# zju3dv/EnvGS

Measured on AMD Instinct MI355X. Metric: train iters/s (fwd+bwd of the render hot path + Adam step, one 800x800 view per GPU per iter) + render Mpix/s, higher is better.
Workload: dtype f32

## Files before the change

envgs_amd/_lib.py:

```python
import ctypes
import os

import torch

HERE = os.path.dirname(os.path.abspath(__file__))
LIB_PATH = os.path.join(HERE, "libenvgs_hip.so")
_lib = None

c_void_p, c_int, c_uint32, c_size_t = ctypes.c_void_p, ctypes.c_int, ctypes.c_uint32, ctypes.c_size_t


class RasterCfg(ctypes.Structure):
    _fields_ = [("P", ctypes.c_int32), ("sh_degree", ctypes.c_int32), ("sh_coeffs", ctypes.c_int32),
                ("channels", ctypes.c_int32), ("width", ctypes.c_int32), ("height", ctypes.c_int32),
                ("bg_len", ctypes.c_int32), ("debug", ctypes.c_int32), ("scale_modifier", ctypes.c_float),
                ("tanfovx", ctypes.c_float), ("tanfovy", ctypes.c_float), ("feature_f16", ctypes.c_int32)]


class AdamTensor(ctypes.Structure):
    _fields_ = [("param", ctypes.c_void_p), ("grad", ctypes.c_void_p), ("exp_avg", ctypes.c_void_p), ("exp_avg_sq", ctypes.c_void_p),
                ("numel", ctypes.c_int64), ("lr", ctypes.c_float), ("step", ctypes.c_float)]


class RowsTensor(ctypes.Structure):
    _fields_ = [("src", ctypes.c_void_p), ("dst", ctypes.c_void_p), ("row_bytes", ctypes.c_int64)]


class GrowTensor(ctypes.Structure):
    _fields_ = [("src", ctypes.c_void_p), ("dst", ctypes.c_void_p), ("row_bytes", ctypes.c_int64), ("kind", ctypes.c_int32), ("reserved0", ctypes.c_int32)]


class DensifyPlanArgs(ctypes.Structure):
    _fields_ = ([("P", ctypes.c_int64), ("N", ctypes.c_int32), ("flags", ctypes.c_uint32)]
                + [(n, ctypes.c_float) for n in ("grad_threshold", "size_limit", "split_screen_threshold", "min_opacity", "min_gradient", "r")]
                + [(n, ctypes.c_void_p) for n in ("ga", "dn", "mr", "wa", "scal", "opac", "cls", "scan", "counters", "temp")]
                + [("temp_bytes", ctypes.c_size_t)])


class DensifyRewriteArgs(ctypes.Structure):
    _fields_ = ([("P", ctypes.c_int64), ("out_rows", ctypes.c_int64), ("n_samples", ctypes.c_int64), ("N", ctypes.c_int32), ("count", ctypes.c_int32),
                 ("ratio_n", ctypes.c_double), ("r", ctypes.c_float), ("reserved0", ctypes.c_uint32)]
                + [(n, ctypes.c_void_p) for n in ("cls", "scan", "counters", "scal", "rotation", "samples")]
                + [("tensors", ctypes.POINTER(GrowTensor))])


class TraceLists(ctypes.Structure):
    _fields_ = [("hit_lists", ctypes.c_void_p), ("hit_cnt", ctypes.c_void_p), ("n_used", ctypes.c_void_p), ("cap", ctypes.c_int32),
                ("surf_acc", ctypes.c_void_p), ("surf_cnt", ctypes.c_void_p), ("surf_off", ctypes.c_void_p),
                ("scan_temp", ctypes.c_void_p), ("scan_temp_bytes", ctypes.c_size_t), ("ray_keys", ctypes.c_void_p),
                ("ray_order", ctypes.c_void_p), ("ray_sort_temp", ctypes.c_void_p), ("ray_sort_temp_bytes", ctypes.c_size_t),
                ("records", ctypes.c_void_p),
                ("num_records", ctypes.c_uint64), ("hit_state", ctypes.c_void_p), ("entries", ctypes.c_void_p), ("pairs", ctypes.c_void_p),
                ("n_entries", ctypes.c_void_p), ("compact_rows", ctypes.c_uint64), ("row_off", ctypes.c_void_p), ("batch_rows", ctypes.c_void_p),
                ("row_blk", ctypes.c_void_p), ("sh_perm", ctypes.c_void_p), ("state_planes", ctypes.c_int32),
                ("sparse_hits", ctypes.c_void_p), ("sparse_cap", ctypes.c_uint64),
                ("defer_reduce", ctypes.c_uint32), ("reserved0", ctypes.c_uint32), ("bwd_order", ctypes.c_void_p)]


class TraceCfg(ctypes.Structure):
    _fields_ = [("P", ctypes.c_int32), ("num_rays", ctypes.c_int32), ("sh_degree", ctypes.c_int32),
                ("sh_coeffs", ctypes.c_int32), ("max_trace_depth", ctypes.c_int32), ("start_from_first", ctypes.c_int32),
                ("has_others", ctypes.c_int32), ("bg_len", ctypes.c_int32), ("debug", ctypes.c_int32),
                ("ray_h", ctypes.c_int32), ("ray_w", ctypes.c_int32),
                ("scale_modifier", ctypes.c_float), ("specular_threshold", ctypes.c_float), ("feature_f16", ctypes.c_int32)]


class SupervisorArgs(ctypes.Structure):
    _fields_ = ([("N", ctypes.c_int64), ("P", ctypes.c_int64), ("flags", ctypes.c_uint32), ("reserved0", ctypes.c_uint32),
                 ("weight", ctypes.c_float * 5), ("reserved1", ctypes.c_float)]
                + [(n, ctypes.c_void_p) for n in ("norm_map", "surf_norm_map", "acc_map", "dpt_map", "dist_map", "env_opacity", "prior", "msk", "R", "near_far")]
                + [(n, ctypes.c_int64) for n in ("norm_map_row", "norm_map_ch", "surf_norm_map_row", "surf_norm_map_ch", "acc_map_row", "dpt_map_row",
                                                 "dist_map_row", "env_opacity_row", "prior_row", "prior_ch", "msk_row")]
                + [(n, ctypes.c_void_p) for n in ("g_norm_map", "g_surf_norm_map", "g_acc_map", "g_dist_map", "g_env_opacity", "partial")])


class SurfelInputsArgs(ctypes.Structure):
    _fields_ = ([(n, ctypes.c_int32) for n in ("P", "sh_degree", "sh_coeffs", "spec_channels")]
                + [(n, ctypes.c_void_p) for n in ("xyz", "features_dc", "features_rest", "scaling", "rotation", "opacity", "specular", "roughness", "campos",
                                                  "scales", "rotations", "opacities", "specular_act", "roughness_act", "shs", "colors", "others", "vertices",
                                                  "clamped",
                                                  "g_scales", "g_rotations", "g_opacities", "g_specular_act", "g_roughness_act", "g_shs", "g_colors", "g_others",
                                                  "d_xyz", "d_features_dc", "d_features_rest", "d_scaling", "d_rotation", "d_opacity", "d_specular", "d_roughness")])


class TsdfVolume(ctypes.Structure):
    _fields_ = ([(n, ctypes.c_int32) for n in ("nx", "ny", "nz")] + [(n, ctypes.c_float) for n in ("ox", "oy", "oz", "voxel")]
                + [(n, ctypes.c_void_p) for n in ("tsdf", "weight", "rgb")])


class TsdfView(ctypes.Structure):
    _fields_ = [("depth", ctypes.c_void_p), ("rgb", ctypes.c_void_p), ("H", ctypes.c_int32), ("W", ctypes.c_int32),
                ("fx", ctypes.c_float), ("fy", ctypes.c_float), ("cx", ctypes.c_float), ("cy", ctypes.c_float),
                ("R", ctypes.c_float * 9), ("T", ctypes.c_float * 3), ("depth_max", ctypes.c_float), ("trunc", ctypes.c_float)]


class TsdfViews(ctypes.Structure):
    _fields_ = [("count", ctypes.c_int32), ("reserved0", ctypes.c_int32), ("v", TsdfView * 8)]


_P = c_void_p
SYMBOLS = {
    "envgs_raster_scan_temp_bytes": (c_size_t, [ctypes.c_int32]),
    "envgs_raster_sort_temp_bytes": (c_size_t, [c_uint32, ctypes.c_int32, ctypes.c_int32]),
    "envgs_raster_project": (c_int, [ctypes.POINTER(RasterCfg)] + [_P] * 15 + [_P, c_size_t, ctypes.POINTER(c_uint32), _P]),
    "envgs_raster_bin_and_render": (c_int, [ctypes.POINTER(RasterCfg), c_uint32] + [_P] * 7 + [_P, c_size_t] + [_P] * 7 + [_P]),
    "envgs_raster_render_audit": (c_int, [ctypes.POINTER(RasterCfg)] + [_P] * 11 + [ctypes.c_int32, _P, _P]),
    "envgs_raster_backward": (c_int, [ctypes.POINTER(RasterCfg), c_uint32] + [_P] * 29 + [_P]),
    "envgs_bvh_temp_bytes": (c_size_t, [ctypes.c_int32]),
    "envgs_bvh_node_floats": (c_size_t, [ctypes.c_int32]),
    "envgs_bvh_build": (c_int, [ctypes.c_int32, _P, _P, _P, _P, c_size_t, ctypes.c_int32, _P]),
    "envgs_bvh_refit": (c_int, [ctypes.c_int32, _P, _P, _P, _P, _P, c_size_t, ctypes.c_int32, _P]),
    "envgs_bvh_quality": (c_int, [ctypes.c_int32, _P, _P, _P]),
    "envgs_trace_ray_sort_temp_bytes": (c_size_t, [ctypes.c_int32]),
    "envgs_trace_ray_order": (c_int, [ctypes.c_int32, _P, _P, _P, ctypes.c_int32, _P, _P, _P, c_size_t, _P]),
    "envgs_trace_forward": (c_int, [ctypes.POINTER(TraceCfg)] + [_P] * 22 + [ctypes.POINTER(TraceLists), _P]),
    "envgs_trace_backward": (c_int, [ctypes.POINTER(TraceCfg)] + [_P] * 35 + [ctypes.POINTER(TraceLists), _P]),
    "envgs_trace_backward_join": (c_int, [_P]),
    "envgs_sh_colors_forward": (c_int, [ctypes.c_int32] * 4 + [_P] * 7 + [_P]),
    "envgs_sh_colors_backward": (c_int, [ctypes.c_int32] * 4 + [_P] * 9 + [_P]),
    "envgs_surfel_quads": (c_int, [ctypes.c_int32] + [_P] * 5 + [_P]),
    "envgs_blend_forward": (c_int, [ctypes.c_int32] * 3 + [_P] * 3 + [_P]),
    "envgs_blend_backward": (c_int, [ctypes.c_int32] * 3 + [_P] * 5 + [_P]),
    "envgs_bounce_rays_forward": (c_int, [ctypes.c_int32] + [_P] * 8 + [_P]),
    "envgs_bounce_rays_backward": (c_int, [ctypes.c_int32] + [_P] * 13 + [_P]),
    "envgs_bounce_blend_forward": (c_int, [ctypes.c_int32] + [_P] * 5 + [_P]),
    "envgs_bounce_blend_backward": (c_int, [ctypes.c_int32] + [_P] * 8 + [_P]),
    "envgs_bounce_pack_mid": (c_int, [ctypes.c_int32, _P, ctypes.c_int32, ctypes.c_int32] + [_P] * 8 + [_P]),
    "envgs_reflect_forward": (c_int, [ctypes.c_int32, ctypes.c_int32, ctypes.c_float] + [_P] * 8 + [_P]),
    "envgs_reflect_backward": (c_int, [ctypes.c_int32, ctypes.c_int32, ctypes.c_float] + [_P] * 11 + [_P]),
    "envgs_select_acc": (c_int, [ctypes.c_int32, ctypes.c_int32, ctypes.c_float, _P, _P, _P]),
    "envgs_reflect_filtered_forward": (c_int, [ctypes.c_int32, ctypes.c_int32, ctypes.c_float, ctypes.c_int32] + [_P] * 10 + [_P]),
    "envgs_reflect_filtered_backward": (c_int, [ctypes.c_int32, ctypes.c_int32, ctypes.c_float, ctypes.c_int32] + [_P] * 13 + [_P]),
    "envgs_blend_filtered_forward": (c_int, [ctypes.c_int32] * 4 + [_P] * 6 + [_P]),
    "envgs_blend_filtered_backward": (c_int, [ctypes.c_int32] * 4 + [_P] * 7 + [_P]),
    "envgs_surface_normal_forward": (c_int, [ctypes.c_int32, ctypes.c_int32, ctypes.c_float, ctypes.c_float, ctypes.c_float] + [_P] * 4 + [_P]),
    "envgs_surface_normal_backward": (c_int, [ctypes.c_int32, ctypes.c_int32, ctypes.c_float, ctypes.c_float, ctypes.c_float] + [_P] * 5 + [_P]),
    "envgs_surfel_inputs_forward": (c_int, [ctypes.POINTER(SurfelInputsArgs), _P]),
    "envgs_surfel_inputs_backward": (c_int, [ctypes.POINTER(SurfelInputsArgs), _P]),
    "envgs_fused_adam": (c_int, [ctypes.c_int32, ctypes.POINTER(AdamTensor), ctypes.c_float, ctypes.c_float, ctypes.c_float, _P]),
    "envgs_compact_temp_bytes": (ctypes.c_size_t, [ctypes.c_int64]),
    "envgs_compact_scan": (c_int, [ctypes.c_int64, _P, _P, _P, _P, ctypes.c_size_t, _P]),
    "envgs_compact_gather": (c_int, [ctypes.c_int32, ctypes.POINTER(RowsTensor), ctypes.c_int64, _P, _P, _P]),
    "envgs_compact_gather_rows": (c_int, [ctypes.c_int32, ctypes.POINTER(RowsTensor), ctypes.c_int64, ctypes.c_int64, _P, _P, _P]),
    "envgs_knn3_mean_dist2": (c_int, [ctypes.c_int32, _P, _P, _P]),
    "envgs_densify_stats": (c_int, [ctypes.c_int64, ctypes.c_int32] + [_P] * 8 + [_P]),
    "envgs_densify_plan_temp_bytes": (ctypes.c_size_t, [ctypes.c_int64]),
    "envgs_densify_plan": (c_int, [ctypes.POINTER(DensifyPlanArgs), _P]),
    "envgs_densify_split_stds": (c_int, [ctypes.c_int64, ctypes.c_int32] + [_P] * 5 + [ctypes.c_int64, _P]),
    "envgs_densify_rewrite": (c_int, [ctypes.POINTER(DensifyRewriteArgs), _P]),
    "envgs_weight_select_temp_bytes": (ctypes.c_size_t, []),
    "envgs_weight_select": (c_int, [ctypes.c_int64, _P, _P, ctypes.c_int32, ctypes.c_int64, ctypes.c_int64, _P, _P, _P, ctypes.c_size_t, _P]),
    "envgs_visibility_mask_temp_bytes": (ctypes.c_size_t, [ctypes.c_int64]),
    "envgs_visibility_mask": (c_int, [ctypes.c_int64, _P, _P, ctypes.c_int64, _P, _P, _P, _P, ctypes.c_size_t, _P]),
    "envgs_oversize_plan": (c_int, [ctypes.c_int64, c_uint32, ctypes.c_float, ctypes.c_float] + [_P] * 8 + [_P]),
    "envgs_tsdf_integrate": (c_int, [ctypes.POINTER(TsdfVolume), ctypes.POINTER(TsdfViews), ctypes.c_float, _P]),
    "envgs_mesh_temp_bytes": (c_size_t, [ctypes.c_int32] * 3),
    "envgs_mesh_count": (c_int, [ctypes.POINTER(TsdfVolume), ctypes.c_float, ctypes.c_float, _P, c_size_t, _P, _P]),
    "envgs_mesh_extract": (c_int, [ctypes.POINTER(TsdfVolume), ctypes.c_float, _P, c_size_t, c_uint32, c_uint32, _P, _P, _P, _P]),
    "envgs_mesh_components_temp_bytes": (c_size_t, [c_uint32, c_uint32]),
    "envgs_mesh_components": (c_int, [c_uint32, c_uint32, _P, _P, c_size_t] + [_P] * 5 + [_P]),
    "envgs_mesh_select_temp_bytes": (c_size_t, [c_uint32, c_uint32]),
    "envgs_mesh_select_count": (c_int, [c_uint32, c_uint32, _P, _P, _P, c_size_t, _P, _P]),
    "envgs_mesh_select_emit": (c_int, [c_uint32, c_uint32] + [_P] * 4 + [_P, c_size_t, c_uint32, c_uint32] + [_P] * 4 + [_P]),
    "envgs_l1_ssim_partial_count": (ctypes.c_int64, [ctypes.c_int32, ctypes.c_int32, ctypes.c_int32]),
    "envgs_l1_ssim_forward": (c_int, [ctypes.c_int32, ctypes.c_int32, ctypes.c_int32, _P, _P, _P, _P, _P]),
    "envgs_l1_ssim_backward": (c_int, [ctypes.c_int32, ctypes.c_int32, ctypes.c_int32, _P, _P, _P, _P, ctypes.c_float, ctypes.c_float, _P, _P]),
    "envgs_depth_percentiles_temp_bytes": (c_size_t, []),
    "envgs_depth_percentiles": (c_int, [ctypes.c_int64, _P, ctypes.c_int64, _P, _P, c_size_t, _P]),
    "envgs_supervisor_partial_count": (ctypes.c_int64, [ctypes.c_int64, ctypes.c_int64]),
    "envgs_supervisor_forward": (c_int, [ctypes.POINTER(SupervisorArgs), _P]),
    "envgs_supervisor_finish": (c_int, [ctypes.POINTER(SupervisorArgs), _P, _P]),
    "envgs_supervisor_backward": (c_int, [ctypes.c_int64, _P, _P, _P, _P]),
    "envgs_debug_set": (None, [ctypes.c_int32, ctypes.c_int32]),
    "envgs_debug_get": (ctypes.c_int32, [ctypes.c_int32]),
    "envgs_prof_enable": (None, [c_int]),
    "envgs_prof_select": (None, [ctypes.c_uint64]),
    "envgs_prof_read": (c_int, [c_int, ctypes.POINTER(ctypes.c_double), ctypes.POINTER(c_int)]),
    "envgs_prof_kernel_name": (ctypes.c_char_p, [c_int]),
}


LIB_DIAG_PATH = os.path.join(HERE, "libenvgs_hip_diag.so")
_libs = {}
_selected = {"kind": "product"}


def _open(path):
    if not os.path.exists(path):
        raise RuntimeError(
            "envgs_amd: %s is missing. Build it with `python -m envgs_amd.build` (hipcc, gfx950). "
            "There is no CPU fallback for the render-and-trace path." % path)
    lib = ctypes.CDLL(path)
    for name, (res, args) in SYMBOLS.items():
        fn = getattr(lib, name)
        fn.restype = res
        fn.argtypes = args
    return lib


def load():
    global _lib
    kind = _selected["kind"]
    lib = _libs.get(kind)
    if lib is None:
        lib = _libs[kind] = _open(LIB_PATH if kind == "product" else LIB_DIAG_PATH)
    _lib = lib
    return lib


def select(kind):
    if kind not in ("product", "diag"):
        raise ValueError(kind)
    old = _selected["kind"]
    _selected["kind"] = kind
    load()
    return old


def ptr(t):
    return None if t is None else ctypes.c_void_p(t.data_ptr())


def check(rc, what):
    if rc != 0:
        raise RuntimeError("envgs_amd: %s failed with code %d (%s)" % (
            what, rc, {-1: "bad argument", -2: "temp buffer too small"}.get(rc, "hipError_t")))
```

envgs_amd/csrc/common.h:

```cpp
#pragma once
#include <hip/hip_runtime.h>
#include <hip/hip_fp16.h>
#include <stdint.h>

#include "../../include/envgs_raster.h"
#include "prof.h"

namespace envgs {

constexpr int TILE = ENVGS_TILE;
constexpr int GEOM = ENVGS_GEOM_STRIDE;
constexpr int GREC = ENVGS_GRAD_STRIDE;
constexpr float NEAR_N = 0.2f;
constexpr float FAR_N = 100.0f;
constexpr float FILTER_SIZE = 0.707106f;
constexpr float FILTER_INV_SQ = 2.0f;
constexpr float ALPHA_CAP = 0.99f;
constexpr float ALPHA_MIN = 1.0f / 255.0f;
constexpr float T_EPS = 0.0001f;

struct Feat {
    const void *p;
    bool h;
    __device__ __forceinline__ float operator[](size_t i) const {
        return h ? __half2float(reinterpret_cast<const __half *>(p)[i]) : reinterpret_cast<const float *>(p)[i];
    }
    __device__ __forceinline__ Feat at(size_t i) const { return Feat{reinterpret_cast<const char *>(p) + i * (h ? 2 : 4), h}; }
};

#define ENVGS_CHECK_LAUNCH(cfg, stream)                                             \
    do {                                                                            \
        hipError_t e__ = hipGetLastError();                                         \
        if (e__ != hipSuccess) return (int)e__;                                     \
        if ((cfg)->debug) {                                                         \
            e__ = hipStreamSynchronize((hipStream_t)(stream));                      \
            if (e__ != hipSuccess) return (int)e__;                                 \
        }                                                                           \
    } while (0)

template <int CTRL, int ROW_MASK = 0xf, int BANK_MASK = 0xf, bool BOUND = true>
__device__ __forceinline__ float dpp_mov(float v) {
    return __builtin_bit_cast(float, __builtin_amdgcn_update_dpp(0, __builtin_bit_cast(int, v), CTRL, ROW_MASK, BANK_MASK, BOUND));
}

__device__ __forceinline__ float wave_sum(float v) {
    v += dpp_mov<0xB1>(v);
    v += dpp_mov<0x4E>(v);
    v += dpp_mov<0x141>(v);
    v += dpp_mov<0x140>(v);
    v += dpp_mov<0x142, 0xa, 0xf, false>(v);
    v += dpp_mov<0x143, 0xc, 0xf, false>(v);
    return __builtin_bit_cast(float, __builtin_amdgcn_readlane(__builtin_bit_cast(int, v), 63));
}


typedef unsigned envgs_u2 __attribute__((ext_vector_type(2)));

__device__ __forceinline__ float wave_reduce64(const float (&g)[64], const int lane)
{
    float z[32];
#pragma unroll
    for (int i = 0; i < 32; i++) {
        const envgs_u2 r = __builtin_amdgcn_permlane32_swap(__float_as_uint(g[i]), __float_as_uint(g[i + 32]), false, false);
        z[i] = __uint_as_float(r.x) + __uint_as_float(r.y);
    }
    float w[16];
#pragma unroll
    for (int k = 0; k < 16; k++) {
        const envgs_u2 q = __builtin_amdgcn_permlane16_swap(__float_as_uint(z[k]), __float_as_uint(z[k + 16]), false, false);
        w[k] = __uint_as_float(q.x) + __uint_as_float(q.y);
    }
    const bool b3 = lane & 8, b2 = lane & 4, b1 = lane & 2, b0 = lane & 1;
    float a[8];
#pragma unroll
    for (int k = 0; k < 8; k++) a[k] = (b3 ? w[k + 8] : w[k]) + dpp_mov<0x140>(b3 ? w[k] : w[k + 8]);
    float b[4];
#pragma unroll
    for (int k = 0; k < 4; k++) b[k] = (b2 ? a[k + 4] : a[k]) + dpp_mov<0x141>(b2 ? a[k] : a[k + 4]);
    float c[2];
#pragma unroll
    for (int k = 0; k < 2; k++) c[k] = (b1 ? b[k + 2] : b[k]) + dpp_mov<0x1B>(b1 ? b[k] : b[k + 2]);
    return (b0 ? c[1] : c[0]) + dpp_mov<0xB1>(b0 ? c[0] : c[1]);
}

template <int CTRL, int ROW_MASK = 0xf>
__device__ __forceinline__ float dpp_fill(float v, float ident) {
    return __builtin_bit_cast(float, __builtin_amdgcn_update_dpp(__builtin_bit_cast(int, ident), __builtin_bit_cast(int, v), CTRL, ROW_MASK, 0xf, false));
}
__device__ __forceinline__ float wave_scan_add(float v) {
    v += dpp_fill<0x111>(v, 0.f); v += dpp_fill<0x112>(v, 0.f); v += dpp_fill<0x114>(v, 0.f); v += dpp_fill<0x118>(v, 0.f);
    v += dpp_fill<0x142, 0xa>(v, 0.f);
    v += dpp_fill<0x143, 0xc>(v, 0.f);
    return v;
}
__device__ __forceinline__ float wave_scan_mul(float v) {
    v *= dpp_fill<0x111>(v, 1.f); v *= dpp_fill<0x112>(v, 1.f); v *= dpp_fill<0x114>(v, 1.f); v *= dpp_fill<0x118>(v, 1.f);
    v *= dpp_fill<0x142, 0xa>(v, 1.f);
    v *= dpp_fill<0x143, 0xc>(v, 1.f);
    return v;
}
__device__ __forceinline__ float wave_bcast(float v, int l) { return __builtin_bit_cast(float, __builtin_amdgcn_readlane(__builtin_bit_cast(int, v), l)); }

template <int N4>
__device__ __forceinline__ float wave_transpose_reduce(const float (&g)[4 * N4], const int lane)
{
    float z[2 * N4];
#pragma unroll
    for (int i = 0; i < 2 * N4; i++) {
        const envgs_u2 r = __builtin_amdgcn_permlane32_swap(__float_as_uint(g[i]), __float_as_uint(g[i + 2 * N4]), false, false);
        z[i] = __uint_as_float(r.x) + __uint_as_float(r.y);
    }
    float w[N4];
#pragma unroll
    for (int k = 0; k < N4; k++) {
        const envgs_u2 q = __builtin_amdgcn_permlane16_swap(__float_as_uint(z[k]), __float_as_uint(z[k + N4]), false, false);
        float v = __uint_as_float(q.x) + __uint_as_float(q.y);
        v += dpp_mov<0x128>(v);
        v += dpp_mov<0x124>(v);
        v += dpp_mov<0x122>(v);
        v += dpp_mov<0x121>(v);
        w[k] = v;
    }
    float out = w[0];
#pragma unroll
    for (int k = 1; k < N4; k++) out = ((lane & 15) == k) ? w[k] : out;
    return out;
}

__device__ __forceinline__ int lane_id() { return __builtin_amdgcn_mbcnt_hi(~0u, __builtin_amdgcn_mbcnt_lo(~0u, 0u)); }

__device__ __forceinline__ void atomic_add_f32(float *p, float v) { unsafeAtomicAdd(p, v); }

int launch_project(const envgs_raster_cfg *cfg, const float *means3D, const float *scales, const float *rotations,
                   const float *opacities, const float *shs, const float *transmat_precomp, const float *viewmatrix,
                   const float *projmatrix, const float *campos, float *geom, float *rgb, uint8_t *clamped,
                   int32_t *radii, uint32_t *tiles_touched, hipStream_t stream);
int launch_scan(const uint32_t *in, uint32_t *out, int n, void *temp, size_t temp_bytes, hipStream_t stream);
size_t scan_temp_bytes(int n);
size_t sort_temp_bytes(uint32_t n, int width, int height);
int launch_bin(const envgs_raster_cfg *cfg, uint32_t N, const float *geom, const int32_t *radii, uint64_t *tile_pairs,
               uint64_t *keys_sorted, uint32_t *point_list, void *bin_temp, size_t bin_temp_bytes, uint32_t *ranges, hipStream_t stream);
size_t key_sort_temp_bytes(int n);
int launch_key_sort(int n, const uint64_t *keys_in, uint64_t *keys_out, int top_bit, void *temp, size_t temp_bytes, hipStream_t stream);
size_t ray_sort_temp_bytes(int R);
int launch_ray_sort(int R, const float *ray_o, const float *ray_d, const float4 *nodes, int P, uint64_t *pairs, uint32_t *order, void *temp,
                    size_t temp_bytes, hipStream_t stream);
int launch_render_fwd(const envgs_raster_cfg *cfg, const uint32_t *ranges, const uint32_t *point_list, const float *geom,
                      const float *colors, const float *bg, float *out_color, float *allmap, float *final_T,
                      int32_t *n_contrib, float *weight, hipStream_t stream, uint8_t *audit_contrib = nullptr, int audit_lmax = 0, int colors_f16 = 0,
                      uint8_t *contrib_mask = nullptr, const uint8_t *audit_skip = nullptr);
int launch_render_bwd(const envgs_raster_cfg *cfg, const uint32_t *ranges, const uint32_t *point_list, const float *geom,
                      const float *colors, const float *bg, const float *final_T, const int32_t *n_contrib,
                      const float *dL_dcolor, const float *dL_dallmap, float *grad_rec, hipStream_t stream, int colors_f16 = 0,
                      const uint8_t *contrib_mask = nullptr);
int launch_project_bwd(const envgs_raster_cfg *cfg, const float *geom, const float *means3D, const float *scales,
                       const float *rotations, const float *shs, const uint8_t *clamped, const float *transmat_precomp,
                       const int32_t *radii, const float *viewmatrix, const float *projmatrix, const float *campos,
                       const float *grad_rec, float *dmeans3D, float *dmeans2D, float *dscales, float *drots, float *dshs,
                       float *dcolors, float *dopacities, float *dtransmat_precomp, hipStream_t stream);

int launch_sh_record_bwd(int P, int D, const float *means3D, const float *shs, const float *campos, const uint8_t *clamped, const int32_t *radii,
                         const float *grad_rec, float *dmeans3D, float *dshs, hipStream_t stream);

__host__ __device__ inline int tile_bits(int width, int height) {
    int tiles = ((width + TILE - 1) / TILE) * ((height + TILE - 1) / TILE);
    int b = 0;
    while ((1 << b) < tiles) b++;
    return b < 1 ? 1 : b;
}

}
```

envgs_amd/csrc/raster_api.hip:

```cpp
#include "common.h"

using namespace envgs;

extern "C" {

size_t envgs_raster_scan_temp_bytes(int32_t P) { return scan_temp_bytes(P); }

size_t envgs_raster_sort_temp_bytes(uint32_t N, int32_t width, int32_t height)
{
    return sort_temp_bytes(N, width, height);
}

static int check_cfg(const envgs_raster_cfg *cfg)
{
    if (!cfg) return ENVGS_ERR_BAD_ARG;
    if (cfg->channels != 3 && cfg->channels != 5 && cfg->channels != 7) return ENVGS_ERR_BAD_ARG;
    if (cfg->sh_degree < 0 || cfg->sh_degree > 3) return ENVGS_ERR_BAD_ARG;
    if (cfg->width <= 0 || cfg->height <= 0 || cfg->P < 0) return ENVGS_ERR_BAD_ARG;
    return 0;
}

int envgs_raster_project(const envgs_raster_cfg *cfg, const float *means3D, const float *scales, const float *rotations,
                         const float *opacities, const float *shs, const float *transmat_precomp,
                         const float *viewmatrix, const float *projmatrix, const float *campos, float *geom, float *rgb,
                         uint8_t *clamped, int32_t *radii, uint32_t *tiles_touched, uint32_t *offsets, void *scan_temp,
                         size_t scan_temp_bytes_, uint32_t *num_rendered_host, void *stream_)
{
    int rc = check_cfg(cfg);
    if (rc) return rc;
    if (num_rendered_host) *num_rendered_host = 0;
    if (cfg->P == 0) return 0;
    if (!means3D || !opacities || !viewmatrix || !projmatrix || !geom || !radii || !tiles_touched || !offsets) return ENVGS_ERR_BAD_ARG;
    if (!transmat_precomp && (!scales || !rotations)) return ENVGS_ERR_BAD_ARG;
    if (shs && (cfg->channels != 3 || !rgb || !clamped || !campos || cfg->sh_coeffs < (cfg->sh_degree + 1) * (cfg->sh_degree + 1))) return ENVGS_ERR_BAD_ARG;
    hipStream_t stream = (hipStream_t)stream_;
    rc = launch_project(cfg, means3D, scales, rotations, opacities, shs, transmat_precomp, viewmatrix, projmatrix, campos,
                        geom, rgb, clamped, radii, tiles_touched, stream);
    if (rc) return rc;
    if (scan_temp_bytes_ < scan_temp_bytes(cfg->P)) return ENVGS_ERR_TEMP_TOO_SMALL;
    rc = launch_scan(tiles_touched, offsets, cfg->P, scan_temp, scan_temp_bytes_, stream);
    if (rc) return rc;
    if (!num_rendered_host) return 0;
    hipError_t e = hipMemcpyAsync(num_rendered_host, offsets + (cfg->P - 1), sizeof(uint32_t), hipMemcpyDeviceToHost, stream);
    if (e != hipSuccess) return (int)e;
    e = hipStreamSynchronize(stream);
    return (int)e;
}

int envgs_raster_bin_and_render(const envgs_raster_cfg *cfg, uint32_t N, const float *geom, const int32_t *radii,
                                const float *colors, const float *bg, uint64_t *tile_pairs, uint64_t *keys_sorted, uint32_t *point_list,
                                void *bin_temp, size_t bin_temp_bytes_, uint32_t *ranges, float *out_color, float *allmap,
                                float *final_T, int32_t *n_contrib, float *weight, uint8_t *contrib_mask, void *stream_)
{
    int rc = check_cfg(cfg);
    if (rc) return rc;
    if (!ranges || !out_color || !allmap || !final_T || !n_contrib || !bg) return ENVGS_ERR_BAD_ARG;
    if (cfg->P > 0 && (!geom || !radii || !colors || !weight)) return ENVGS_ERR_BAD_ARG;
    if (N > 0 && (!tile_pairs || !point_list || !bin_temp)) return ENVGS_ERR_BAD_ARG;
    hipStream_t stream = (hipStream_t)stream_;
    rc = launch_bin(cfg, N, geom, radii, tile_pairs, keys_sorted, point_list, bin_temp, bin_temp_bytes_, ranges, stream);
    if (rc) return rc;
    return launch_render_fwd(cfg, ranges, point_list, geom, colors, bg, out_color, allmap, final_T, n_contrib, weight, stream, nullptr, 0,
                             (cfg->feature_f16 && cfg->sh_coeffs == 0) ? 1 : 0, contrib_mask);
}

int envgs_raster_render_audit(const envgs_raster_cfg *cfg, const float *geom, const float *colors, const float *bg,
                              const uint32_t *point_list, const uint32_t *ranges, float *out_color, float *allmap, float *final_T,
                              int32_t *n_contrib, float *weight, uint8_t *contrib, int32_t lmax, const uint8_t *skip_px, void *stream_)
{
    int rc = check_cfg(cfg);
    if (rc) return rc;
    if (!ranges || !out_color || !allmap || !final_T || !n_contrib || !bg || !contrib || lmax <= 0) return ENVGS_ERR_BAD_ARG;
    if (cfg->P > 0 && (!geom || !colors || !weight || !point_list)) return ENVGS_ERR_BAD_ARG;
    hipStream_t stream = (hipStream_t)stream_;
    hipError_t e = hipMemsetAsync(contrib, 0, (size_t)cfg->width * cfg->height * (size_t)lmax, stream);
    if (e != hipSuccess) return (int)e;
    return launch_render_fwd(cfg, ranges, point_list, geom, colors, bg, out_color, allmap, final_T, n_contrib, weight, stream, contrib, lmax,
                             (cfg->feature_f16 && cfg->sh_coeffs == 0) ? 1 : 0, nullptr, skip_px);
}

int envgs_raster_backward(const envgs_raster_cfg *cfg, uint32_t N, const float *geom, const float *colors, const float *bg,
                          const uint32_t *point_list, const uint32_t *ranges, const float *final_T,
                          const int32_t *n_contrib, const uint8_t *contrib_mask, const float *dL_dcolor, const float *dL_dallmap, const float *means3D,
                          const float *scales, const float *rotations, const float *shs, const uint8_t *clamped,
                          const float *transmat_precomp, const int32_t *radii, const float *viewmatrix,
                          const float *projmatrix, const float *campos, float *grad_rec, float *dmeans3D, float *dmeans2D,
                          float *dscales, float *drots, float *dshs, float *dcolors, float *dopacities,
                          float *dtransmat_precomp, void *stream_)
{
    int rc = check_cfg(cfg);
    if (rc) return rc;
    if (cfg->P == 0) return 0;
    if (!geom || !colors || !bg || !ranges || !final_T || !n_contrib || !grad_rec || !radii ||
        !dmeans2D || !dopacities || !viewmatrix || !projmatrix)
        return ENVGS_ERR_BAD_ARG;
    if (N > 0 && !point_list) return ENVGS_ERR_BAD_ARG;
    if (shs ? (!dshs || !clamped || !campos || !means3D) : !dcolors) return ENVGS_ERR_BAD_ARG;
    if (transmat_precomp ? !dtransmat_precomp : (!scales || !rotations || !means3D || !dmeans3D || !dscales || !drots)) return ENVGS_ERR_BAD_ARG;
    hipStream_t stream = (hipStream_t)stream_;
    rc = launch_render_bwd(cfg, ranges, point_list, geom, colors, bg, final_T, n_contrib, dL_dcolor, dL_dallmap, grad_rec, stream,
                           (cfg->feature_f16 && !shs) ? 1 : 0, contrib_mask);
    if (rc) return rc;
    return launch_project_bwd(cfg, geom, means3D, scales, rotations, shs, clamped, transmat_precomp, radii, viewmatrix,
                              projmatrix, campos, grad_rec, dmeans3D, dmeans2D, dscales, drots, dshs, dcolors, dopacities,
                              dtransmat_precomp, stream);
}

}
```

envgs_amd/csrc/raster_bin.hip:

```cpp
#include "common.h"
#include "ray_key.h"
#include "tile_sort.h"

namespace envgs {

template <int CTRL, int ROW_MASK = 0xf>
__device__ __forceinline__ uint32_t dpp_fill_u32(uint32_t v) {
    return (uint32_t)__builtin_amdgcn_update_dpp(0, (int)v, CTRL, ROW_MASK, 0xf, false);
}
__device__ __forceinline__ uint32_t wave_scan_add_u32(uint32_t v) {
    v += dpp_fill_u32<0x111>(v); v += dpp_fill_u32<0x112>(v); v += dpp_fill_u32<0x114>(v); v += dpp_fill_u32<0x118>(v);
    v += dpp_fill_u32<0x142, 0xa>(v);
    v += dpp_fill_u32<0x143, 0xc>(v);
    return v;
}

template <int NW>
__device__ __forceinline__ uint32_t block_exclusive_u32(uint32_t v, uint32_t *s_w, uint32_t &total)
{
    const int lane = lane_id(), wave = threadIdx.x >> 6;
    const uint32_t inc = wave_scan_add_u32(v);
    if (lane == 63) s_w[wave] = inc;
    __syncthreads();
    uint32_t before = 0, all = 0;
#pragma unroll
    for (int k = 0; k < NW; k++) { const uint32_t t = s_w[k]; all += t; before += (k < wave) ? t : 0u; }
    total = all;
    __syncthreads();
    return before + inc - v;
}

constexpr int SCAN_ITEMS = 1024;

size_t scan_temp_bytes(int n) { return sizeof(uint32_t) * (size_t)(((n > 0 ? n : 1) + SCAN_ITEMS - 1) / SCAN_ITEMS) + 64; }

__global__ void __launch_bounds__(256)
scan_block_sums(const uint32_t *__restrict__ in, uint32_t *__restrict__ sums, int n)
{
    __shared__ uint32_t s_w[5];
    const int base = blockIdx.x * SCAN_ITEMS + threadIdx.x * 4;
    uint32_t s = 0;
#pragma unroll
    for (int k = 0; k < 4; k++) s += (base + k < n) ? in[base + k] : 0u;
    uint32_t total;
    (void)block_exclusive_u32<4>(s, s_w, total);
    if (threadIdx.x == 0) sums[blockIdx.x] = total;
}

__global__ void __launch_bounds__(256)
scan_apply(const uint32_t *in, uint32_t *out, const uint32_t *__restrict__ sums, int n)
{
    __shared__ uint32_t s_w[5];
    uint32_t pre = 0;
    for (int k = threadIdx.x; k < (int)blockIdx.x; k += 256) pre += sums[k];
    uint32_t before;
    (void)block_exclusive_u32<4>(pre, s_w, before);
    const int base = blockIdx.x * SCAN_ITEMS + threadIdx.x * 4;
    uint32_t a[4];
#pragma unroll
    for (int k = 0; k < 4; k++) a[k] = (base + k < n) ? in[base + k] : 0u;
    a[1] += a[0]; a[2] += a[1]; a[3] += a[2];
    uint32_t total;
    const uint32_t ex = block_exclusive_u32<4>(a[3], s_w, total) + before;
#pragma unroll
    for (int k = 0; k < 4; k++) if (base + k < n) out[base + k] = ex + a[k];
}

int launch_scan(const uint32_t *in, uint32_t *out, int n, void *temp, size_t temp_bytes, hipStream_t stream)
{
    if (n <= 0) return 0;
    if (temp_bytes < scan_temp_bytes(n)) return ENVGS_ERR_TEMP_TOO_SMALL;
    ProfScope prof_(K_SCAN, stream);
    const int nb = (n + SCAN_ITEMS - 1) / SCAN_ITEMS;
    hipLaunchKernelGGL(scan_block_sums, dim3(nb), dim3(256), 0, stream, in, (uint32_t *)temp, n);
    hipLaunchKernelGGL(scan_apply, dim3(nb), dim3(256), 0, stream, in, out, (const uint32_t *)temp, n);
    return (int)hipGetLastError();
}

constexpr int BIN_ROWS_MAX = 512;
constexpr int BIN_SLICE_MIN = 1024;
constexpr int BIN_BAND = 16384;
constexpr int BIG_RECT = 32;
constexpr int SORT_LONG_N = 16384;
constexpr int SORT_LONG_WGS = 256;

struct BinPlan { int rows, slice, ntiles; };
static BinPlan bin_plan(int P, int W, int H)
{
    BinPlan p;
    p.ntiles = ((W + TILE - 1) / TILE) * ((H + TILE - 1) / TILE);
    int rows = (P + BIN_SLICE_MIN - 1) / BIN_SLICE_MIN;
    rows = rows < 1 ? 1 : (rows > BIN_ROWS_MAX ? BIN_ROWS_MAX : rows);
    p.slice = (((P + rows - 1) / rows + 255) / 256) * 256;
    p.rows = p.slice > 0 ? (P + p.slice - 1) / p.slice : 1;
    if (p.rows < 1) p.rows = 1;
    return p;
}

size_t sort_temp_bytes(uint32_t, int width, int height)
{
    const size_t ntiles = (size_t)((width + TILE - 1) / TILE) * ((height + TILE - 1) / TILE);
    return sizeof(uint32_t) * ((size_t)BIN_ROWS_MAX * ntiles + 3 * ntiles + 1 + 4) + 256;
}

__device__ __forceinline__ bool tile_rect(int i, int W, int H, const float *__restrict__ geom, const int32_t *__restrict__ radii,
                                          int &x0, int &y0, int &x1, int &y1, uint32_t &dbits)
{
    const int rad = radii[i];
    if (rad <= 0) return false;
    const float cx = geom[(size_t)i * GEOM + 9], cy = geom[(size_t)i * GEOM + 10];
    dbits = __float_as_uint(geom[(size_t)i * GEOM + 15]);
    const float radius = (float)rad;
    const int gx = (W + TILE - 1) / TILE, gy = (H + TILE - 1) / TILE;
    x0 = (int)((cx - radius) / (float)TILE); x0 = x0 < 0 ? 0 : (x0 > gx ? gx : x0);
    y0 = (int)((cy - radius) / (float)TILE); y0 = y0 < 0 ? 0 : (y0 > gy ? gy : y0);
    x1 = (int)((cx + radius + (float)(TILE - 1)) / (float)TILE); x1 = x1 < 0 ? 0 : (x1 > gx ? gx : x1);
    y1 = (int)((cy + radius + (float)(TILE - 1)) / (float)TILE); y1 = y1 < 0 ? 0 : (y1 > gy ? gy : y1);
    return x1 > x0 && y1 > y0;
}

struct SurfelRect { int x0, y0, x1, y1; uint32_t dbits; bool vis; };
__device__ __forceinline__ SurfelRect load_rect(int i, int g1, int W, int H, const float *__restrict__ geom, const int32_t *__restrict__ radii)
{
    SurfelRect r;
    r.x0 = r.y0 = r.x1 = r.y1 = 0; r.dbits = 0;
    r.vis = i < g1 && tile_rect(i, W, H, geom, radii, r.x0, r.y0, r.x1, r.y1, r.dbits);
    return r;
}

template <bool SCATTER>
__global__ void __launch_bounds__(256)
bin_pass(int P, int W, int H, int slice, int ntiles, const float *__restrict__ geom, const int32_t *__restrict__ radii,
         uint32_t *hist, const uint32_t *__restrict__ tile_start, uint64_t *__restrict__ pairs, uint32_t cap)
{
    extern __shared__ uint32_t s_bin[];
    const int gx = (W + TILE - 1) / TILE;
    const int g0 = blockIdx.x * slice, g1 = min(P, g0 + slice);
    uint32_t *row = hist + (size_t)blockIdx.x * ntiles;
    const int lane = lane_id();
    for (int band0 = 0; band0 < ntiles; band0 += BIN_BAND) {
        const int bn = min(BIN_BAND, ntiles - band0);
        SurfelRect cur = load_rect(g0 + (int)threadIdx.x, g1, W, H, geom, radii);
        for (int t = threadIdx.x; t < bn; t += 256) s_bin[t] = SCATTER ? tile_start[band0 + t] + row[band0 + t] : 0u;
        __syncthreads();
        auto visit = [&](int t, uint64_t pair) {
            t -= band0;
            if ((unsigned)t >= (unsigned)bn) return;
            const uint32_t slot = atomicAdd(&s_bin[t], 1u);
            if (SCATTER && slot < cap) pairs[slot] = pair;
        };
        for (int ib = g0; ib < g1; ib += 256) {
            const int i = ib + (int)threadIdx.x;
            const SurfelRect c = cur;
            cur = load_rect(i + 256, g1, W, H, geom, radii);
            const int x0 = c.x0, y0 = c.y0, x1 = c.x1, y1 = c.y1;
            const uint32_t dbits = c.dbits;
            const bool vis = c.vis;
            const uint64_t pair = ((uint64_t)dbits << 32) | (uint32_t)i;
            const bool big = vis && (x1 - x0) * (y1 - y0) > BIG_RECT;
            if (vis && !big)
                for (int y = y0; y < y1; y++)
                    for (int x = x0; x < x1; x++) visit(y * gx + x, pair);
            uint64_t m = __builtin_amdgcn_ballot_w64(big);
            while (m) {
                const int l = __builtin_ctzll(m);
                m &= m - 1;
                const int bx0 = __builtin_amdgcn_readlane(x0, l), by0 = __builtin_amdgcn_readlane(y0, l);
                const int bw = __builtin_amdgcn_readlane(x1, l) - bx0, bh = __builtin_amdgcn_readlane(y1, l) - by0;
                const uint64_t bp = ((uint64_t)(uint32_t)__builtin_amdgcn_readlane((int)dbits, l) << 32) | (uint32_t)__builtin_amdgcn_readlane(i, l);
                for (int k = lane; k < bw * bh; k += 64) visit((by0 + k / bw) * gx + bx0 + k % bw, bp);
            }
        }
        __syncthreads();
        if (!SCATTER)
            for (int t = threadIdx.x; t < bn; t += 256) row[band0 + t] = s_bin[t];
        __syncthreads();
    }
}

constexpr int CS_SEG = 16, CS_ROWS = BIN_ROWS_MAX / CS_SEG;
__global__ void __launch_bounds__(256)
bin_column_scan(int rows, int ntiles, uint32_t *hist, uint32_t *__restrict__ tile_count)
{
    __shared__ uint32_t s_seg[CS_SEG][16];
    const int tl = threadIdx.x & 15, seg = threadIdx.x >> 4;
    const int t = blockIdx.x * 16 + tl;
    const int per = (rows + CS_SEG - 1) / CS_SEG, r0 = seg * per;
    uint32_t v[CS_ROWS];
    uint32_t s = 0;
#pragma unroll
    for (int k = 0; k < CS_ROWS; k++) {
        const int r = r0 + k;
        v[k] = (t < ntiles && k < per && r < rows) ? hist[(size_t)r * ntiles + t] : 0u;
        s += v[k];
    }
    s_seg[seg][tl] = s;
    __syncthreads();
    uint32_t acc = 0;
#pragma unroll
    for (int k = 0; k < CS_SEG; k++) acc += (k < seg) ? s_seg[k][tl] : 0u;
    if (t >= ntiles) return;
#pragma unroll
    for (int k = 0; k < CS_ROWS; k++) {
        const int r = r0 + k;
        if (k < per && r < rows) hist[(size_t)r * ntiles + t] = acc;
        acc += v[k];
    }
    if (seg == CS_SEG - 1) tile_count[t] = acc;
}

__global__ void __launch_bounds__(1024)
bin_tile_scan(int ntiles, const uint32_t *__restrict__ tile_count, uint32_t *__restrict__ tile_start, uint32_t *__restrict__ ranges,
              uint32_t cap, uint32_t *__restrict__ hdr)
{
    __shared__ uint32_t s_w[17];
    const int per = (ntiles + 1023) / 1024, b = min(ntiles, (int)threadIdx.x * per), e = min(ntiles, b + per);
    uint32_t s = 0;
    for (int k = b; k < e; k++) s += tile_count[k];
    uint32_t total;
    uint32_t run = block_exclusive_u32<16>(s, s_w, total);
    const bool ok = total <= cap;
    for (int k = b; k < e; k++) {
        const uint32_t c = tile_count[k];
        tile_start[k] = run;
        ranges[2 * k] = (c && ok) ? run : 0u;
        ranges[2 * k + 1] = (c && ok) ? run + c : 0u;
        run += c;
    }
    if (threadIdx.x == 0) { tile_start[ntiles] = total; hdr[0] = total; hdr[1] = 0u; hdr[2] = 0u; hdr[3] = 0u; }
}

template <int NT>
__device__ __forceinline__ void sort_padded_lds(uint64_t *s, int lp, int tid)
{
    const int npad = 1 << lp;
    for (int g = tid; g < (npad >> TS_S); g += NT) bitonic_first(s, g, lp);
    __syncthreads();
    for (int lk = TS_S + 1; lk <= lp; lk++)
        for (int a = lk - 1; a >= 0;) {
            const int S = ts_chunk(a);
            if (S == 4) { for (int g = tid; g < (npad >> 4); g += NT) bitonic_group<4>(s, g, lk, a, lp); }
            else if (S == 3) { for (int g = tid; g < (npad >> 3); g += NT) bitonic_group<3>(s, g, lk, a, lp); }
            else if (S == 2) { for (int g = tid; g < (npad >> 2); g += NT) bitonic_group<2>(s, g, lk, a, lp); }
            else { for (int g = tid; g < (npad >> 1); g += NT) bitonic_group<1>(s, g, lk, a, lp); }
            __syncthreads();
            a -= S;
        }
}

template <int NT>
__device__ __forceinline__ void merge_padded_lds(uint64_t *s, int lc, int tid)
{
    const int npad = 1 << lc;
    for (int a = lc - 1; a >= 0;) {
        const int S = ts_chunk(a);
        if (S == 4) { for (int g = tid; g < (npad >> 4); g += NT) bitonic_group<4>(s, g, lc, a, lc); }
        else if (S == 3) { for (int g = tid; g < (npad >> 3); g += NT) bitonic_group<3>(s, g, lc, a, lc); }
        else if (S == 2) { for (int g = tid; g < (npad >> 2); g += NT) bitonic_group<2>(s, g, lc, a, lc); }
        else { for (int g = tid; g < (npad >> 1); g += NT) bitonic_group<1>(s, g, lc, a, lc); }
        __syncthreads();
        a -= S;
    }
}

constexpr int lds_slots(int lp_cap) { return (1 << lp_cap) + (1 << (lp_cap - 5)); }

__device__ __forceinline__ void store_sorted(uint64_t v, uint32_t tile, size_t at, uint64_t *keys_sorted, uint32_t *point_list, int full64)
{
    if (full64) { keys_sorted[at] = v; return; }
    point_list[at] = (uint32_t)v;
    if (keys_sorted) keys_sorted[at] = ((uint64_t)tile << 32) | (v >> 32);
}

template <int NT>
__device__ __forceinline__ void load_sort_write(uint64_t *s, const uint64_t *pairs, int n, uint32_t tile, uint32_t b,
                                                uint64_t *keys_sorted, uint32_t *point_list, int tid, int full64)
{
    const int lp = ts_log2_padded(n);
    for (int i = tid; i < (1 << lp); i += NT) s[ts_slot(i)] = i < n ? pairs[b + i] : ~0ull;
    __syncthreads();
    sort_padded_lds<NT>(s, lp, tid);
    for (int i = tid; i < n; i += NT) store_sorted(s[ts_slot(i)], tile, (size_t)b + i, keys_sorted, point_list, full64);
}

template <int LP_CAP, int NT>
__global__ void __launch_bounds__(NT)
sort_tile_lists(const uint32_t *__restrict__ ranges, const uint64_t *pairs, uint64_t *keys_sorted, uint32_t *__restrict__ point_list,
                uint32_t *__restrict__ hdr, uint32_t *__restrict__ long_list, int full64)
{
    __shared__ uint64_t s_k[lds_slots(LP_CAP)];
    const uint32_t t = blockIdx.x, b = ranges[2 * t];
    const int n = (int)(ranges[2 * t + 1] - b);
    if (n == 0) return;
    if (n > (1 << LP_CAP)) {
        if (threadIdx.x == 0) long_list[atomicAdd(&hdr[1], 1u)] = t;
        return;
    }
    load_sort_write<NT>(s_k, pairs, n, t, b, keys_sorted, point_list, (int)threadIdx.x, full64);
}

constexpr int LONG_ITEM = 4096;
constexpr int LONG_BATCH = 256;

__device__ __forceinline__ uint32_t long_claim(uint32_t *hdr, uint32_t *s_item)
{
    __syncthreads();
    if (threadIdx.x == 0) *s_item = atomicAdd(&hdr[2], 1u);
    __syncthreads();
    return *s_item;
}
__device__ __forceinline__ void long_wait(uint32_t *hdr, const uint32_t base)
{
    if (threadIdx.x == 0)
        while (__hip_atomic_load(&hdr[3], __ATOMIC_ACQUIRE, __HIP_MEMORY_SCOPE_AGENT) < base) __builtin_amdgcn_s_sleep(4);
    __syncthreads();
    __threadfence();
}
__device__ __forceinline__ void long_done(uint32_t *hdr)
{
    __threadfence();
    __syncthreads();
    if (threadIdx.x == 0) __hip_atomic_fetch_add(&hdr[3], 1u, __ATOMIC_RELEASE, __HIP_MEMORY_SCOPE_AGENT);
}

__global__ void __launch_bounds__(1024)
sort_long_lists(const uint32_t *__restrict__ ranges, uint64_t *pairs, uint64_t *keys_sorted, uint32_t *__restrict__ point_list,
                uint32_t *hdr, const uint32_t *__restrict__ long_list, int full64)
{
    __shared__ uint64_t s_long[lds_slots(14)];
    __shared__ uint32_t s_item;
    __shared__ uint32_t s_bt[LONG_BATCH], s_bb[LONG_BATCH], s_bn[LONG_BATCH], s_pref[LONG_BATCH + 1];
    const uint32_t count = hdr[1];
    const int tid = (int)threadIdx.x, G = (int)gridDim.x;
    constexpr int LC = 14, C = 1 << LC;
    const bool copy_out = !(full64 && keys_sorted == pairs);
    uint32_t small_seen = 0u, big = 0u;
    for (uint32_t w = 0; w < count; w++) {
        const uint32_t t = long_list[w], b = ranges[2 * t];
        const int n = (int)(ranges[2 * t + 1] - b);
        if (n > SORT_LONG_N) { big++; continue; }
        if ((small_seen++ % (uint32_t)G) != blockIdx.x) continue;
        load_sort_write<1024>(s_long, pairs, n, t, b, keys_sorted, point_list, tid, full64);
        __syncthreads();
    }
    if (big == 0u) return;
    auto lp_of = [&](const int n) { int lp = LC; while ((1 << lp) < n) lp++; return lp; };
    auto items_of = [&](const int kind, const int lk, const int n) -> uint32_t {
        const int lp = lp_of(n);
        if (kind == 1) return lk <= lp ? (uint32_t)(((1ll << (lp - 1)) + LONG_ITEM - 1) / LONG_ITEM) : 0u;
        return (kind == 2 || lk <= lp) ? (uint32_t)((n + C - 1) / C) : 0u;
    };
    auto do_item = [&](const int kind, const int lk, const int q, const int l, const uint32_t it) {
        const uint32_t t = s_bt[l], b = s_bb[l];
        const int n = (int)s_bn[l];
        uint64_t *seg = pairs + b;
        if (kind == 0) {
            const int c = (int)it;
            for (int i = tid; i < C; i += 1024) s_long[ts_slot(i)] = ((long long)c * C + i) < n ? seg[(size_t)c * C + i] : ~0ull;
            __syncthreads();
            if (lk == LC) sort_padded_lds<1024>(s_long, LC, tid);
            else merge_padded_lds<1024>(s_long, LC, tid);
            for (int i = tid; i < C; i += 1024)
                if ((long long)c * C + i < n) seg[(size_t)c * C + i] = s_long[ts_slot(i)];
        } else if (kind == 1) {
            const int lp = lp_of(n);
            const long long i0 = (long long)it * LONG_ITEM, i1 = min(i0 + LONG_ITEM, 1ll << (lp - 1));
            for (long long idx = i0 + tid; idx < i1; idx += 1024) ascending_step(seg, n, lk, q, (int)idx);
        } else {
            const long long i0 = (long long)it * C, i1 = min(i0 + C, (long long)n);
            for (long long i = i0 + tid; i < i1; i += 1024) store_sorted(seg[i], t, (size_t)b + (size_t)i, keys_sorted, point_list, full64);
        }
    };
    uint32_t base = 0u, my = long_claim(hdr, &s_item);
    uint32_t w = 0;
    while (w < count) {
        __syncthreads();
        int nl = 0, lp_max = LC;
        for (; w < count && nl < LONG_BATCH; w++) {
            const uint32_t t = long_list[w], b = ranges[2 * t];
            const int n = (int)(ranges[2 * t + 1] - b);
            if (n <= SORT_LONG_N) continue;
            if (tid == 0) { s_bt[nl] = t; s_bb[nl] = b; s_bn[nl] = (uint32_t)n; }
            lp_max = max(lp_max, lp_of(n));
            nl++;
        }
        if (nl == 0) break;
        auto run_phase = [&](const int kind, const int lk, const int q) {
            __syncthreads();
            if (tid < nl) {
                uint32_t acc = 0u;
                for (int l = 0; l < tid; l++) acc += items_of(kind, lk, (int)s_bn[l]);
                s_pref[tid] = acc;
                if (tid == nl - 1) s_pref[nl] = acc + items_of(kind, lk, (int)s_bn[tid]);
            }
            __syncthreads();
            const uint32_t items = s_pref[nl];
            while (my - base < items) {
                const uint32_t j = my - base;
                int lo = 0, hi = nl - 1;
                while (lo < hi) { const int mid = (lo + hi + 1) >> 1; if (s_pref[mid] <= j) lo = mid; else hi = mid - 1; }
                long_wait(hdr, base);
                do_item(kind, lk, q, lo, j - s_pref[lo]);
                long_done(hdr);
                my = long_claim(hdr, &s_item);
            }
            base += items;
        };
        run_phase(0, LC, 0);
        for (int lk = LC + 1; lk <= lp_max; lk++) {
            for (int q = 0; q <= lk - LC - 1; q++) run_phase(1, lk, q);
            run_phase(0, lk, 0);
        }
        if (copy_out) run_phase(2, 0, 0);
    }
}

static int long_sort_grid()
{
    static int cached[16] = {};
    int dev = 0;
    if (hipGetDevice(&dev) != hipSuccess || dev < 0 || dev >= 16) return 64;
    if (cached[dev] == 0) {
        int cus = 0;
        if (hipDeviceGetAttribute(&cus, hipDeviceAttributeMultiprocessorCount, dev) != hipSuccess || cus <= 0) cus = 64;
        cached[dev] = cus < SORT_LONG_WGS ? cus : SORT_LONG_WGS;
    }
    return cached[dev];
}

int launch_bin(const envgs_raster_cfg *cfg, uint32_t N, const float *geom, const int32_t *radii, uint64_t *tile_pairs,
               uint64_t *keys_sorted, uint32_t *point_list, void *bin_temp, size_t bin_temp_bytes, uint32_t *ranges, hipStream_t stream)
{
    const BinPlan pl = bin_plan(cfg->P, cfg->width, cfg->height);
    if (N == 0 || cfg->P <= 0) return (int)hipMemsetAsync(ranges, 0, sizeof(uint32_t) * 2 * (size_t)pl.ntiles, stream);
    if (bin_temp_bytes < sort_temp_bytes(N, cfg->width, cfg->height)) return ENVGS_ERR_TEMP_TOO_SMALL;
    uint32_t *hist = (uint32_t *)bin_temp;
    uint32_t *tile_count = hist + (size_t)BIN_ROWS_MAX * pl.ntiles;
    uint32_t *tile_start = tile_count + pl.ntiles;
    uint32_t *long_list = tile_start + pl.ntiles + 1;
    uint32_t *hdr = long_list + pl.ntiles;
    const size_t lds = sizeof(uint32_t) * (size_t)(pl.ntiles < BIN_BAND ? pl.ntiles : BIN_BAND);
    prof_begin(K_EMIT_KEYS, stream);
    hipLaunchKernelGGL(bin_pass<false>, dim3(pl.rows), dim3(256), lds, stream, cfg->P, cfg->width, cfg->height, pl.slice, pl.ntiles,
                       geom, radii, hist, (const uint32_t *)nullptr, (uint64_t *)nullptr, 0u);
    ENVGS_CHECK_LAUNCH(cfg, stream);
    hipLaunchKernelGGL(bin_column_scan, dim3((pl.ntiles + 15) / 16), dim3(256), 0, stream, pl.rows, pl.ntiles, hist, tile_count);
    ENVGS_CHECK_LAUNCH(cfg, stream);
    hipLaunchKernelGGL(bin_tile_scan, dim3(1), dim3(1024), 0, stream, pl.ntiles, tile_count, tile_start, ranges, N, hdr);
    ENVGS_CHECK_LAUNCH(cfg, stream);
    hipLaunchKernelGGL(bin_pass<true>, dim3(pl.rows), dim3(256), lds, stream, cfg->P, cfg->width, cfg->height, pl.slice, pl.ntiles,
                       geom, radii, hist, tile_start, tile_pairs, N);
    ENVGS_CHECK_LAUNCH(cfg, stream);
    prof_end(K_EMIT_KEYS, stream);
    ProfScope prof_(K_SORT, stream);
    const uint64_t want = (uint64_t)N * 8 / ((uint64_t)pl.ntiles * 5);
    if (want <= 2048)
        hipLaunchKernelGGL((sort_tile_lists<11, 128>), dim3(pl.ntiles), dim3(128), 0, stream, ranges, tile_pairs, keys_sorted, point_list, hdr, long_list, 0);
    else if (want <= 4096)
        hipLaunchKernelGGL((sort_tile_lists<12, 256>), dim3(pl.ntiles), dim3(256), 0, stream, ranges, tile_pairs, keys_sorted, point_list, hdr, long_list, 0);
    else
        hipLaunchKernelGGL((sort_tile_lists<13, 512>), dim3(pl.ntiles), dim3(512), 0, stream, ranges, tile_pairs, keys_sorted, point_list, hdr, long_list, 0);
    ENVGS_CHECK_LAUNCH(cfg, stream);
    hipLaunchKernelGGL(sort_long_lists, dim3(long_sort_grid()), dim3(1024), 0, stream, ranges, tile_pairs,
                       keys_sorted, point_list, hdr, long_list, 0);
    ENVGS_CHECK_LAUNCH(cfg, stream);
    return 0;
}

static void launch_bucket_sorts(uint64_t n, int nb, const uint32_t *ranges, uint64_t *pairs, uint64_t *keys_sorted, uint32_t *point_list,
                                uint32_t *hdr, uint32_t *long_list, int full64, hipStream_t stream)
{
    const uint64_t want = n * 8 / ((uint64_t)nb * 5);
    if (want <= 2048)
        hipLaunchKernelGGL((sort_tile_lists<11, 128>), dim3(nb), dim3(128), 0, stream, ranges, pairs, keys_sorted, point_list, hdr, long_list, full64);
    else if (want <= 4096)
        hipLaunchKernelGGL((sort_tile_lists<12, 256>), dim3(nb), dim3(256), 0, stream, ranges, pairs, keys_sorted, point_list, hdr, long_list, full64);
    else
        hipLaunchKernelGGL((sort_tile_lists<13, 512>), dim3(nb), dim3(512), 0, stream, ranges, pairs, keys_sorted, point_list, hdr, long_list, full64);
    hipLaunchKernelGGL(sort_long_lists, dim3(long_sort_grid()), dim3(1024), 0, stream, ranges, pairs, keys_sorted, point_list, hdr, long_list, full64);
}

static int ray_bucket_bits(int R)
{
    int b = 4;
    while (b < 13 && ((long long)160 << b) < R) b++;
    return b;
}

size_t ray_sort_temp_bytes(int R)
{
    const size_t nb = (size_t)1 << ray_bucket_bits(R);
    return sizeof(uint32_t) * ((size_t)BIN_ROWS_MAX * nb + 5 * nb + 1 + 4 + (size_t)(R > 0 ? R : 1) + 6 * (size_t)BIN_ROWS_MAX) + 256;
}

__global__ void __launch_bounds__(256)
ray_origin_bounds(int R, int slice, const float *__restrict__ ray_o, float *__restrict__ partial)
{
    __shared__ float s_red[4][6];
    const int g0 = blockIdx.x * slice, g1 = min(R, g0 + slice);
    float lo[3] = {3.0e38f, 3.0e38f, 3.0e38f}, hi[3] = {-3.0e38f, -3.0e38f, -3.0e38f};
    for (int i = g0 + (int)threadIdx.x; i < g1; i += 256) {
#pragma unroll
        for (int c = 0; c < 3; c++) { const float x = ray_o[3 * i + c]; if (x == x && fabsf(x) < 1.0e30f) { lo[c] = fminf(lo[c], x); hi[c] = fmaxf(hi[c], x); } }
    }
#pragma unroll
    for (int c = 0; c < 3; c++)
        for (int o = 32; o > 0; o >>= 1) { lo[c] = fminf(lo[c], __shfl_xor(lo[c], o)); hi[c] = fmaxf(hi[c], __shfl_xor(hi[c], o)); }
    const int wave = threadIdx.x >> 6, lane = threadIdx.x & 63;
    if (lane == 0) { for (int c = 0; c < 3; c++) { s_red[wave][c] = lo[c]; s_red[wave][3 + c] = hi[c]; } }
    __syncthreads();
    if (threadIdx.x < 6) {
        const int c = threadIdx.x;
        float v = s_red[0][c];
        for (int w = 1; w < 4; w++) v = c < 3 ? fminf(v, s_red[w][c]) : fmaxf(v, s_red[w][c]);
        partial[blockIdx.x * 6 + c] = v;
    }
}

template <bool SCATTER>
__global__ void __launch_bounds__(256)
ray_bucket_pass(int R, int slice, int nb, int shift, const float *__restrict__ ray_o, const float *__restrict__ ray_d,
                const float *__restrict__ bounds_partial, int nrows, int lead, uint32_t *__restrict__ keys, uint32_t *hist, const uint32_t *__restrict__ bucket_start,
                uint64_t *__restrict__ pairs)
{
    extern __shared__ uint32_t s_bin[];
    __shared__ float s_box[6];
    const int g0 = blockIdx.x * slice, g1 = min(R, g0 + slice);
    uint32_t *row = hist + (size_t)blockIdx.x * nb;
    for (int t = threadIdx.x; t < nb; t += 256) s_bin[t] = SCATTER ? bucket_start[t] + row[t] : 0u;
    if (!SCATTER && threadIdx.x < 64) {
        const int c = threadIdx.x % 6, j0 = threadIdx.x / 6;
        float v = c < 3 ? 3.0e38f : -3.0e38f;
        if (j0 < 10)
            for (int j = j0; j < nrows; j += 10) { const float x = bounds_partial[j * 6 + c]; v = c < 3 ? fminf(v, x) : fmaxf(v, x); }
        float acc = v;
        for (int k = 1; k < 10; k++) { const float x = __shfl(v, (int)(threadIdx.x % 6) + 6 * k); if (threadIdx.x < 6) acc = c < 3 ? fminf(acc, x) : fmaxf(acc, x); }
        if (threadIdx.x < 6) s_box[c] = acc;
    }
    __syncthreads();
    float lo0 = 0.f, lo1 = 0.f, lo2 = 0.f, s0 = 0.f, s1 = 0.f, s2 = 0.f;
    if (!SCATTER) {
        lo0 = s_box[0]; lo1 = s_box[1]; lo2 = s_box[2];
        const float e0 = s_box[3] - lo0, e1 = s_box[4] - lo1, e2 = s_box[5] - lo2;
        s0 = e0 > 0.f ? 32.0f / e0 : 0.f; s1 = e1 > 0.f ? 32.0f / e1 : 0.f; s2 = e2 > 0.f ? 32.0f / e2 : 0.f;
    }
    for (int i = g0 + (int)threadIdx.x; i < g1; i += 256) {
        uint32_t key;
        if (SCATTER) key = keys[i];
        else keys[i] = key = ray_coherence_key(i, ray_o, ray_d, lo0, lo1, lo2, s0, s1, s2, lead);
        const uint32_t slot = atomicAdd(&s_bin[key >> shift], 1u);
        if (SCATTER) pairs[slot] = ((uint64_t)key << 32) | (uint32_t)i;
    }
    __syncthreads();
    if (!SCATTER)
        for (int t = threadIdx.x; t < nb; t += 256) row[t] = s_bin[t];
}

int launch_ray_sort(int R, const float *ray_o, const float *ray_d, const float4 *nodes, int P, uint64_t *pairs, uint32_t *order,
                    void *temp, size_t temp_bytes, hipStream_t stream)
{
    (void)nodes; (void)P;
    if (R <= 0) return 0;
    if (temp_bytes < ray_sort_temp_bytes(R)) return ENVGS_ERR_TEMP_TOO_SMALL;
    const int bits = ray_bucket_bits(R), nb = 1 << bits, shift = 31 - bits;
    int rows = (R + BIN_SLICE_MIN - 1) / BIN_SLICE_MIN;
    rows = rows < 1 ? 1 : (rows > BIN_ROWS_MAX ? BIN_ROWS_MAX : rows);
    const int slice = (((R + rows - 1) / rows + 255) / 256) * 256;
    rows = (R + slice - 1) / slice;
    uint32_t *hist = (uint32_t *)temp;
    uint32_t *count = hist + (size_t)BIN_ROWS_MAX * nb;
    uint32_t *start = count + nb;
    uint32_t *long_list = start + nb + 1;
    uint32_t *hdr = long_list + nb;
    uint32_t *ranges = hdr + 4;
    uint32_t *keys = ranges + 2 * (size_t)nb;
    float *partial = (float *)(keys + (size_t)R);
    const size_t lds = sizeof(uint32_t) * (size_t)nb;
    int lead = debug_switch(ENVGS_DBG_RAYKEY) > 0 ? debug_switch(ENVGS_DBG_RAYKEY) - 1 : RAY_KEY_LEAD;
    lead = lead > 8 ? 8 : lead;
    hipLaunchKernelGGL(ray_origin_bounds, dim3(rows), dim3(256), 0, stream, R, slice, ray_o, partial);
    hipLaunchKernelGGL(ray_bucket_pass<false>, dim3(rows), dim3(256), lds, stream, R, slice, nb, shift, ray_o, ray_d, (const float *)partial, rows, lead, keys, hist,
                       (const uint32_t *)nullptr, (uint64_t *)nullptr);
    hipLaunchKernelGGL(bin_column_scan, dim3((nb + 15) / 16), dim3(256), 0, stream, rows, nb, hist, count);
    hipLaunchKernelGGL(bin_tile_scan, dim3(1), dim3(1024), 0, stream, nb, count, start, ranges, (uint32_t)R, hdr);
    hipLaunchKernelGGL(ray_bucket_pass<true>, dim3(rows), dim3(256), lds, stream, R, slice, nb, shift, ray_o, ray_d, (const float *)partial, rows, lead, keys, hist, start, pairs);
    launch_bucket_sorts(R, nb, ranges, pairs, (uint64_t *)nullptr, order, hdr, long_list, 0, stream);
    return (int)hipGetLastError();
}

size_t key_sort_temp_bytes(int n)
{
    const size_t nb = (size_t)1 << ray_bucket_bits(n);
    return sizeof(uint32_t) * ((size_t)BIN_ROWS_MAX * nb + 5 * nb + 1 + 4) + 256;
}

template <bool SCATTER>
__global__ void __launch_bounds__(256)
key_bucket_pass(int n, int slice, int nb, int shift, const uint64_t *__restrict__ keys, uint32_t *hist, const uint32_t *__restrict__ bucket_start,
                uint64_t *__restrict__ out)
{
    extern __shared__ uint32_t s_bin[];
    const int g0 = blockIdx.x * slice, g1 = min(n, g0 + slice);
    uint32_t *row = hist + (size_t)blockIdx.x * nb;
    for (int t = threadIdx.x; t < nb; t += 256) s_bin[t] = SCATTER ? bucket_start[t] + row[t] : 0u;
    __syncthreads();
    for (int i = g0 + (int)threadIdx.x; i < g1; i += 256) {
        const uint64_t k = keys[i];
        const uint32_t slot = atomicAdd(&s_bin[(uint32_t)(k >> shift) & (uint32_t)(nb - 1)], 1u);
        if (SCATTER) out[slot] = k;
    }
    __syncthreads();
    if (!SCATTER)
        for (int t = threadIdx.x; t < nb; t += 256) row[t] = s_bin[t];
}

int launch_key_sort(int n, const uint64_t *keys_in, uint64_t *keys_out, int top_bit, void *temp, size_t temp_bytes, hipStream_t stream)
{
    if (n <= 0) return 0;
    if (temp_bytes < key_sort_temp_bytes(n)) return ENVGS_ERR_TEMP_TOO_SMALL;
    const int bits = ray_bucket_bits(n), nb = 1 << bits, shift = top_bit - bits;
    int rows = (n + BIN_SLICE_MIN - 1) / BIN_SLICE_MIN;
    rows = rows < 1 ? 1 : (rows > BIN_ROWS_MAX ? BIN_ROWS_MAX : rows);
    const int slice = (((n + rows - 1) / rows + 255) / 256) * 256;
    rows = (n + slice - 1) / slice;
    uint32_t *hist = (uint32_t *)temp;
    uint32_t *count = hist + (size_t)BIN_ROWS_MAX * nb;
    uint32_t *start = count + nb;
    uint32_t *long_list = start + nb + 1;
    uint32_t *hdr = long_list + nb;
    uint32_t *ranges = hdr + 4;
    const size_t lds = sizeof(uint32_t) * (size_t)nb;
    hipLaunchKernelGGL(key_bucket_pass<false>, dim3(rows), dim3(256), lds, stream, n, slice, nb, shift, keys_in, hist, (const uint32_t *)nullptr, (uint64_t *)nullptr);
    hipLaunchKernelGGL(bin_column_scan, dim3((nb + 15) / 16), dim3(256), 0, stream, rows, nb, hist, count);
    hipLaunchKernelGGL(bin_tile_scan, dim3(1), dim3(1024), 0, stream, nb, count, start, ranges, (uint32_t)n, hdr);
    hipLaunchKernelGGL(key_bucket_pass<true>, dim3(rows), dim3(256), lds, stream, n, slice, nb, shift, keys_in, hist, start, keys_out);
    launch_bucket_sorts((uint64_t)n, nb, ranges, keys_out, keys_out, (uint32_t *)nullptr, hdr, long_list, 1, stream);
    return (int)hipGetLastError();
}

}
```

envgs_amd/csrc/raster_render.hip:

```cpp
#include "common.h"

namespace envgs {

struct Hit {
    float sx, sy, inv, kx, ky, kz, lx, ly, lz, rho3d, rho2d, dx, dy, depth, G, alpha;
    bool ok;
};

template <bool EXACT>
__device__ __forceinline__ float recip(float x)
{
    if (EXACT) return 1.0f / x;
    const float r = __builtin_amdgcn_rcpf(x);
    return __builtin_fmaf(__builtin_fmaf(-x, r, 1.0f), r, r);
}
template <bool EXACT>
__device__ __forceinline__ float recip1(float x) { return EXACT ? 1.0f / x : __builtin_amdgcn_rcpf(x); }
template <bool EXACT>
__device__ __forceinline__ float expneg(float x) { return EXACT ? expf(x) : __expf(x); }

template <bool EXACT = false>
__device__ __forceinline__ Hit eval_splat(const float4 r0, const float4 r1, const float4 r2, const float4 r3, float px, float py)
{
    Hit h;
    const float Tux = r0.x, Tuy = r0.y, Tuz = r0.z, Tvx = r0.w, Tvy = r1.x, Tvz = r1.y, Twx = r1.z, Twy = r1.w, Twz = r2.x;
    const float cx = r2.y, cy = r2.z, opa = r3.z;
    h.kx = __builtin_fmaf(px, Twx, -Tux); h.ky = __builtin_fmaf(px, Twy, -Tuy); h.kz = __builtin_fmaf(px, Twz, -Tuz);
    h.lx = __builtin_fmaf(py, Twx, -Tvx); h.ly = __builtin_fmaf(py, Twy, -Tvy); h.lz = __builtin_fmaf(py, Twz, -Tvz);
    const float ppx = __builtin_fmaf(h.ky, h.lz, -(h.kz * h.ly));
    const float ppy = __builtin_fmaf(h.kz, h.lx, -(h.kx * h.lz));
    const float ppz = __builtin_fmaf(h.kx, h.ly, -(h.ky * h.lx));
    h.inv = recip<EXACT>(ppz);
    h.sx = ppx * h.inv; h.sy = ppy * h.inv;
    h.rho3d = __builtin_fmaf(h.sx, h.sx, h.sy * h.sy);
    h.dx = cx - px; h.dy = cy - py;
    h.rho2d = FILTER_INV_SQ * __builtin_fmaf(h.dx, h.dx, h.dy * h.dy);
    const bool use3d = h.rho3d <= h.rho2d;
    const float rho = use3d ? h.rho3d : h.rho2d;
    h.depth = use3d ? __builtin_fmaf(h.sx, Twx, __builtin_fmaf(h.sy, Twy, Twz)) : Twz;
    const float power = -0.5f * rho;
    h.G = expneg<EXACT>(power);
    const float a = opa * h.G;
    h.alpha = a < ALPHA_CAP ? a : ALPHA_CAP;
    h.ok = (ppz != 0.0f) && (h.depth >= NEAR_N) && (power <= 0.0f) && (h.alpha >= ALPHA_MIN);
    return h;
}

template <int C, int B = 256>
struct TileLds {
    float4 rec[4][B];
    float col[C][B];
    uint32_t id[B];
    unsigned long long qbits[4][(B + 63) / 64];
};

constexpr int BWD_BATCH = 192;

__device__ __forceinline__ int xcd_tile(int b, int ntiles)
{
    const int per = (ntiles + 7) >> 3;
    return (b & 7) * per + (b >> 3);
}

__device__ __forceinline__ uint32_t quadrant_mask(const float4 r0, const float4 r1, const float4 r2, const float4 r3, int tile_px, int tile_py)
{
    const float Tux = r0.x, Tuy = r0.y, Tuz = r0.z, Tvx = r0.w, Tvy = r1.x, Tvz = r1.y, Twx = r1.z, Twy = r1.w, Twz = r2.x;
    const float cx = r2.y, cy = r2.z, opa = r3.z;
    const float tau = 2.0f * __logf(255.0f * opa);
    if (!(tau >= 0.0f)) return 0u;
    const float r2d = sqrtf(0.5f * tau);
    float bx0 = cx - r2d, bx1 = cx + r2d, by0 = cy - r2d, by1 = cy + r2d;
    const float d = tau * (Twx * Twx + Twy * Twy) - Twz * Twz;
    if (!(d < 0.0f)) return 0xFu;
    const float id = 1.0f / d;
    const float f0 = tau * id, f2 = -id;
    const float pxc = f0 * (Tux * Twx + Tuy * Twy) + f2 * (Tuz * Twz);
    const float pyc = f0 * (Tvx * Twx + Tvy * Twy) + f2 * (Tvz * Twz);
    const float hx = pxc * pxc - (f0 * (Tux * Tux + Tuy * Tuy) + f2 * (Tuz * Tuz));
    const float hy = pyc * pyc - (f0 * (Tvx * Tvx + Tvy * Tvy) + f2 * (Tvz * Tvz));
    const float ex = sqrtf(fmaxf(hx, 0.0f)), ey = sqrtf(fmaxf(hy, 0.0f));
    bx0 = fminf(bx0, pxc - ex); bx1 = fmaxf(bx1, pxc + ex); by0 = fminf(by0, pyc - ey); by1 = fmaxf(by1, pyc + ey);
    const float mx = 0.05f + 1e-3f * (bx1 - bx0), my = 0.05f + 1e-3f * (by1 - by0);
    bx0 -= mx; bx1 += mx; by0 -= my; by1 += my;
    if (!(bx0 <= bx1 && by0 <= by1)) return 0xFu;
    const float ax = Tvy * Twz - Tvz * Twy, ay = Tvz * Twx - Tvx * Twz, az = Tvx * Twy - Tvy * Twx;
    const float bxx = Twy * Tuz - Twz * Tuy, bxy = Twz * Tux - Twx * Tuz, bxz = Twx * Tuy - Twy * Tux;
    const float A00 = ax * ax + ay * ay - tau * az * az, A11 = bxx * bxx + bxy * bxy - tau * bxz * bxz, A01 = ax * bxx + ay * bxy - tau * az * bxz;
    const float det = A00 * A11 - A01 * A01;
    const bool conic = A00 > 0.0f && A11 > 0.0f && det > 1e-6f * A00 * A11 && hx > 0.0f && hy > 0.0f &&
                       fabsf(hx * A00 - hy * A11) <= 0.02f * (hx * A00 + hy * A11);
    const float bound = conic ? 1.05f * hx * det / A11 : 0.0f;
    const float iA00 = conic ? 1.0f / A00 : 0.0f, iA11 = conic ? 1.0f / A11 : 0.0f;
    uint32_t m = 0;
#pragma unroll
    for (int q = 0; q < 4; q++) {
        const float qx = (float)(tile_px + (q & 1) * 8), qy = (float)(tile_py + (q >> 1) * 8);
        if (!(bx0 <= qx + 7.0f && bx1 >= qx && by0 <= qy + 7.0f && by1 >= qy)) continue;
        bool hit = true;
        if (conic) {
            const float ddx = fmaxf(fmaxf(qx - cx, cx - (qx + 7.0f)), 0.0f), ddy = fmaxf(fmaxf(qy - cy, cy - (qy + 7.0f)), 0.0f);
            const bool disc = ddx * ddx + ddy * ddy <= (r2d + 0.05f) * (r2d + 0.05f);
            const float x0 = qx - 0.05f - pxc, x1 = qx + 7.05f - pxc, y0 = qy - 0.05f - pyc, y1 = qy + 7.05f - pyc;
            bool ell = x0 <= 0.0f && x1 >= 0.0f && y0 <= 0.0f && y1 >= 0.0f;
            if (!ell) {
                float fmin = 3.0e38f;
#pragma unroll
                for (int e = 0; e < 2; e++) {
                    const float yy = e ? y1 : y0;
                    const float xs = fminf(fmaxf(-A01 * yy * iA00, x0), x1);
                    fmin = fminf(fmin, (A00 * xs + 2.0f * A01 * yy) * xs + A11 * yy * yy);
                    const float xx = e ? x1 : x0;
                    const float ys = fminf(fmaxf(-A01 * xx * iA11, y0), y1);
                    fmin = fminf(fmin, (A11 * ys + 2.0f * A01 * xx) * ys + A00 * xx * xx);
                }
                ell = fmin <= bound;
            }
            hit = disc || ell || !(bound == bound);
        }
        if (hit) m |= 1u << q;
    }
    return m;
}

template <int C, bool AUDIT, bool EXACT = false>
__global__ void __launch_bounds__(256, 5)
composite_fwd(int W, int H, int bg_len, const uint32_t *__restrict__ ranges, const uint32_t *__restrict__ point_list,
              const float *__restrict__ geom, const Feat colors, const float *__restrict__ bg,
              float *__restrict__ out_color, float *__restrict__ allmap, float *__restrict__ final_T,
              int32_t *__restrict__ n_contrib, float *__restrict__ weight, uint8_t *__restrict__ audit_contrib, int audit_lmax,
              uint8_t *__restrict__ contrib_mask, const uint8_t *__restrict__ audit_skip)
{
    __shared__ TileLds<C> lds;
    __shared__ float wacc[256];
    __shared__ unsigned char cmk[256][4];
    const int gx = (W + TILE - 1) / TILE, gy = (H + TILE - 1) / TILE;
    const int tile = xcd_tile(blockIdx.x, gx * gy);
    if (tile >= gx * gy) return;
    const int tx = tile % gx, ty = tile / gx;
    const int tid = threadIdx.x, wave = tid >> 6, lane = tid & 63;
    const int pxi = tx * TILE + (wave & 1) * 8 + (lane & 7);
    const int pyi = ty * TILE + (wave >> 1) * 8 + (lane >> 3);
    const bool inside = pxi < W && pyi < H;
    const float px = (float)pxi, py = (float)pyi;
    const uint32_t r0 = ranges[2 * tile], r1 = ranges[2 * tile + 1];

    const bool wskip = AUDIT && audit_skip && inside && audit_skip[(size_t)pyi * W + pxi] != 0;
    bool done = !inside;
    float T = 1.0f, Cacc[C], N0 = 0.f, N1 = 0.f, N2 = 0.f, D = 0.f, M1 = 0.f, M2 = 0.f, dist = 0.f, med = 0.f;
    int32_t last = 0, medc = -1;
#pragma unroll
    for (int c = 0; c < C; c++) Cacc[c] = 0.f;
    wacc[tid] = 0.f; reinterpret_cast<unsigned *>(&cmk[0][0])[tid] = 0u;

    for (uint32_t base = r0; base < r1; base += 256) {
        if (__syncthreads_and(done)) break;
        uint32_t qm = 0u;
        if (base + tid < r1) {
            const uint32_t g = point_list[base + tid];
            const float4 *gp = reinterpret_cast<const float4 *>(geom + (size_t)g * GEOM);
            const float4 a0 = gp[0], a1 = gp[1], a2 = gp[2], a3 = gp[3];
            lds.id[tid] = g;
            lds.rec[0][tid] = a0; lds.rec[1][tid] = a1; lds.rec[2][tid] = a2; lds.rec[3][tid] = a3;
            qm = quadrant_mask(a0, a1, a2, a3, tx * TILE, ty * TILE);
#pragma unroll
            for (int c = 0; c < C; c++) lds.col[c][tid] = colors[(size_t)g * C + c];
        }
#pragma unroll
        for (int q = 0; q < 4; q++) {
            const unsigned long long m = __builtin_amdgcn_ballot_w64((qm >> q) & 1u);
            if (lane == 0) lds.qbits[q][wave] = m;
        }
        __syncthreads();
        const int count = (int)min(256u, r1 - base);
        for (int ck = 0; ck * 64 < count && __builtin_amdgcn_ballot_w64(!done) != 0; ck++) {
          unsigned long long todo = lds.qbits[wave][ck];
          todo = ((unsigned long long)(unsigned)__builtin_amdgcn_readfirstlane((int)(todo >> 32)) << 32) | (unsigned)__builtin_amdgcn_readfirstlane((int)todo);
          while (todo != 0ull) {
            const int j = ck * 64 + (int)__builtin_ctzll(todo);
            todo &= todo - 1ull;
            if (__builtin_amdgcn_ballot_w64(!done) == 0) break;
            const Hit h = eval_splat<EXACT>(lds.rec[0][j], lds.rec[1][j], lds.rec[2][j], lds.rec[3][j], px, py);
            bool contrib = !done && h.ok;
            const float test_T = T * (1.0f - h.alpha);
            const bool stop = contrib && test_T < T_EPS;
            done = done || stop;
            contrib = contrib && !stop;
            float w = 0.f;
            if (contrib) {
                const float4 r2 = lds.rec[2][j], r3 = lds.rec[3][j];
                w = h.alpha * T;
                const float A = 1.0f - T;
                const float m = FAR_N / (FAR_N - NEAR_N) * (1.0f - NEAR_N / h.depth);
                dist += (m * m * A + M2 - 2.0f * m * M1) * w;
                D += h.depth * w;
                M1 += m * w;
                M2 += m * m * w;
                const int32_t contributor = (int32_t)(base - r0) + j + 1;
                if (AUDIT) { if (contributor <= audit_lmax) audit_contrib[((size_t)pyi * W + pxi) * (size_t)audit_lmax + (contributor - 1)] = 1; }
                if (T > 0.5f) { med = h.depth; medc = contributor; }
                N0 += r2.w * w; N1 += r3.x * w; N2 += r3.y * w;
#pragma unroll
                for (int c = 0; c < C; c++) Cacc[c] += lds.col[c][j] * w;
                T = test_T;
                last = contributor;
            }
            if (__builtin_amdgcn_ballot_w64(contrib) != 0) {
                const float ws = wave_sum((AUDIT && wskip) ? 0.f : w);
                if (lane == 0) { atomic_add_f32(&wacc[j], ws); cmk[j][wave] = 1; }
            }
          }
        }
        __syncthreads();
        if (tid < count) {
            const float ws = wacc[tid];
            if (ws != 0.0f) { atomic_add_f32(weight + lds.id[tid], ws); wacc[tid] = 0.f; }
            if (contrib_mask) {
                unsigned *cw = reinterpret_cast<unsigned *>(&cmk[0][0]) + tid;
                const unsigned v = *cw;
                contrib_mask[base + tid] = (uint8_t)((v & 1u) | ((v >> 7) & 2u) | ((v >> 14) & 4u) | ((v >> 21) & 8u));
                if (v) *cw = 0u;
            }
        }
    }

    if (inside) {
        const size_t HW = (size_t)H * W, pid = (size_t)pyi * W + pxi;
        final_T[pid] = T; final_T[HW + pid] = M1; final_T[2 * HW + pid] = M2;
        n_contrib[pid] = last; n_contrib[HW + pid] = medc;
#pragma unroll
        for (int c = 0; c < C; c++) out_color[c * HW + pid] = Cacc[c] + T * (c < bg_len ? bg[c] : 0.0f);
        allmap[0 * HW + pid] = D;
        allmap[1 * HW + pid] = 1.0f - T;
        allmap[2 * HW + pid] = N0; allmap[3 * HW + pid] = N1; allmap[4 * HW + pid] = N2;
        allmap[5 * HW + pid] = med;
        allmap[6 * HW + pid] = dist;
    }
}

template <int C, bool DIST, bool EXACT>
__device__ __forceinline__ void composite_bwd_tile(TileLds<C, BWD_BATCH> &lds, float (*gacc)[15 + C], const int W, const int H, const int bg_len,
                                                   const uint32_t *__restrict__ point_list, const float *__restrict__ geom,
                                                   const Feat colors, const float *__restrict__ bg,
                                                   const float *__restrict__ final_T, const int32_t *__restrict__ n_contrib,
                                                   const float *__restrict__ dL_dcolor, const float *__restrict__ dL_dallmap,
                                                   float *__restrict__ grad_rec, const uint32_t r0, const int tx, const int ty, const int max_last,
                                                   const uint8_t *__restrict__ contrib_mask)
{
    constexpr int V = 15 + C;
    constexpr int N4 = (V + 3) / 4;
    const int tid = threadIdx.x, wave = tid >> 6, lane = tid & 63;
    const int pxi = tx * TILE + (wave & 1) * 8 + (lane & 7);
    const int pyi = ty * TILE + (wave >> 1) * 8 + (lane >> 3);
    const bool inside = pxi < W && pyi < H;
    const float px = (float)pxi, py = (float)pyi;
    const size_t HW = (size_t)H * W, pid = (size_t)(inside ? pyi : 0) * W + (inside ? pxi : 0);

    const float T_final = inside ? final_T[pid] : 0.f;
    float T = T_final;
    const int32_t last = inside ? n_contrib[pid] : 0;
    const int32_t medc = inside ? n_contrib[HW + pid] : 0;
    float dpix[C];
    float bg_dot = 0.f;
#pragma unroll
    for (int c = 0; c < C; c++) {
        dpix[c] = (inside && dL_dcolor) ? dL_dcolor[c * HW + pid] : 0.f;
        bg_dot += (c < bg_len ? bg[c] : 0.0f) * dpix[c];
    }
    const float dL_ddepth = (inside && dL_dallmap) ? dL_dallmap[0 * HW + pid] : 0.f;
    const float dL_daccum = (inside && dL_dallmap) ? dL_dallmap[1 * HW + pid] : 0.f;
    const float dL_dn0 = (inside && dL_dallmap) ? dL_dallmap[2 * HW + pid] : 0.f;
    const float dL_dn1 = (inside && dL_dallmap) ? dL_dallmap[3 * HW + pid] : 0.f;
    const float dL_dn2 = (inside && dL_dallmap) ? dL_dallmap[4 * HW + pid] : 0.f;
    const float dL_dmed = (inside && dL_dallmap) ? dL_dallmap[5 * HW + pid] : 0.f;
    const float dL_dreg = (DIST && inside && dL_dallmap) ? dL_dallmap[6 * HW + pid] : 0.f;
    const float final_D = (DIST && inside) ? final_T[HW + pid] : 0.f;
    const float final_D2 = (DIST && inside) ? final_T[2 * HW + pid] : 0.f;
    const float final_A = 1.0f - T_final;
    const float bgT = -T_final * bg_dot;
    float last_alpha = 0.f, lastX = 0.f, accX = 0.f;
    int wmax_last = last;
    wmax_last = max(wmax_last, __shfl_xor(wmax_last, 1)); wmax_last = max(wmax_last, __shfl_xor(wmax_last, 2)); wmax_last = max(wmax_last, __shfl_xor(wmax_last, 4));
    wmax_last = max(wmax_last, __shfl_xor(wmax_last, 8)); wmax_last = max(wmax_last, __shfl_xor(wmax_last, 16)); wmax_last = max(wmax_last, __shfl_xor(wmax_last, 32));
    wmax_last = __builtin_amdgcn_readfirstlane(wmax_last);
    constexpr float MD_A = FAR_N / (FAR_N - NEAR_N), MD_B = (FAR_N * NEAR_N) / (FAR_N - NEAR_N);

    for (int top = max_last; top > 0; top -= BWD_BATCH) {
        __syncthreads();
        uint32_t qm = 0u;
        if (tid < BWD_BATCH && top - 1 - tid >= 0) {
            const uint32_t g = point_list[r0 + (uint32_t)(top - 1 - tid)];
            const float4 *gp = reinterpret_cast<const float4 *>(geom + (size_t)g * GEOM);
            const float4 a0 = gp[0], a1 = gp[1], a2 = gp[2], a3 = gp[3];
            lds.id[tid] = g;
            lds.rec[0][tid] = a0; lds.rec[1][tid] = a1; lds.rec[2][tid] = a2; lds.rec[3][tid] = a3;
            qm = contrib_mask ? (uint32_t)contrib_mask[r0 + (uint32_t)(top - 1 - tid)] : quadrant_mask(a0, a1, a2, a3, tx * TILE, ty * TILE);
#pragma unroll
            for (int c = 0; c < C; c++) lds.col[c][tid] = colors[(size_t)g * C + c];
        }
        if (wave * 64 < BWD_BATCH) {
#pragma unroll
            for (int q = 0; q < 4; q++) {
                const unsigned long long m = __builtin_amdgcn_ballot_w64((qm >> q) & 1u);
                if (lane == 0) lds.qbits[q][wave] = m;
            }
        }
        __syncthreads();
        const int count = min(BWD_BATCH, top);
        const int jmin = max(0, top - wmax_last);
        for (int ck = jmin >> 6; ck * 64 < count; ck++) {
          unsigned long long todo = lds.qbits[wave][ck];
          todo = ((unsigned long long)(unsigned)__builtin_amdgcn_readfirstlane((int)(todo >> 32)) << 32) | (unsigned)__builtin_amdgcn_readfirstlane((int)todo);
          if (ck == (jmin >> 6)) todo &= ~0ull << (jmin & 63);
          while (todo != 0ull) {
            const int j = ck * 64 + (int)__builtin_ctzll(todo);
            todo &= todo - 1ull;
            const int ci = top - 1 - j;
            const bool cand = ci < last;
            if (__builtin_amdgcn_ballot_w64(cand) == 0) continue;
            const float4 q0 = lds.rec[0][j], q1 = lds.rec[1][j], q2 = lds.rec[2][j], q3 = lds.rec[3][j];
            const Hit h = eval_splat<EXACT>(q0, q1, q2, q3, px, py);
            const bool act = cand && h.ok;
            if (__builtin_amdgcn_ballot_w64(act) == 0) continue;

            float gv[4 * N4];
#pragma unroll
            for (int v = 0; v < 4 * N4; v++) gv[v] = 0.f;
            if (act) {
                const float Twx = q1.z, Twy = q1.w, opa = q3.z;
                const float nrm0 = q2.w, nrm1 = q3.x, nrm2 = q3.y;
                const float alpha = h.alpha, G = h.G;
                const float r1 = recip1<EXACT>(1.0f - alpha);
                T = T * r1;
                const float w = alpha * T;
                float X = h.depth * dL_ddepth + dL_daccum;
                X += nrm0 * dL_dn0; X += nrm1 * dL_dn1; X += nrm2 * dL_dn2;
#pragma unroll
                for (int c = 0; c < C; c++) {
                    X += lds.col[c][j] * dpix[c];
                    gv[15 + c] = w * dpix[c];
                }
                float dL_dz = w * dL_ddepth;
                if (ci == medc - 1) dL_dz += dL_dmed;
                if (DIST) {
                    const float idep = recip1<EXACT>(h.depth);
                    const float m_d = MD_A * (1.0f - NEAR_N * idep);
                    X += (final_D2 + m_d * m_d * final_A - 2.0f * m_d * final_D) * dL_dreg;
                    dL_dz += 2.0f * w * (m_d * final_A - final_D) * dL_dreg * (MD_B * idep * idep);
                }
                accX = last_alpha * lastX + (1.f - last_alpha) * accX;
                lastX = X;
                last_alpha = alpha;
                const float dL_dalpha = (X - accX) * T + bgT * r1;
                gv[9] = w * dL_dn0; gv[10] = w * dL_dn1; gv[11] = w * dL_dn2;
                gv[12] = G * dL_dalpha;
                const float nGd = -(opa * dL_dalpha) * G;
                if (h.rho3d <= h.rho2d) {
                    const float dsx = __builtin_fmaf(nGd, h.sx, dL_dz * Twx);
                    const float dsy = __builtin_fmaf(nGd, h.sy, dL_dz * Twy);
                    const float dpx = dsx * h.inv, dpy = dsy * h.inv;
                    const float dpz = -__builtin_fmaf(dpx, h.sx, dpy * h.sy);
                    const float dkx = __builtin_fmaf(h.ly, dpz, -(h.lz * dpy)), dky = __builtin_fmaf(h.lz, dpx, -(h.lx * dpz)), dkz = __builtin_fmaf(h.lx, dpy, -(h.ly * dpx));
                    const float dlx = __builtin_fmaf(dpy, h.kz, -(dpz * h.ky)), dly = __builtin_fmaf(dpz, h.kx, -(dpx * h.kz)), dlz = __builtin_fmaf(dpx, h.ky, -(dpy * h.kx));
                    gv[0] = -dkx; gv[1] = -dky; gv[2] = -dkz;
                    gv[3] = -dlx; gv[4] = -dly; gv[5] = -dlz;
                    gv[6] = __builtin_fmaf(px, dkx, __builtin_fmaf(py, dlx, dL_dz * h.sx));
                    gv[7] = __builtin_fmaf(px, dky, __builtin_fmaf(py, dly, dL_dz * h.sy));
                    gv[8] = __builtin_fmaf(px, dkz, __builtin_fmaf(py, dlz, dL_dz));
                } else {
                    gv[13] = nGd * (FILTER_INV_SQ * h.dx);
                    gv[14] = nGd * (FILTER_INV_SQ * h.dy);
                    gv[8] = dL_dz;
                }
            }
            const float mine = wave_transpose_reduce<N4>(gv, lane);
            const int vi = (lane & 15) + (lane >> 4) * N4;
            if ((lane & 15) < N4 && vi < V) atomic_add_f32(&gacc[j][vi], mine);
          }
        }
        __syncthreads();
        for (int i = tid; i < count * V; i += 256) {
            const int j = i / V, v = i - j * V;
            const float val = gacc[j][v];
            if (val != 0.0f) { atomic_add_f32(grad_rec + (size_t)lds.id[j] * GREC + v, val); gacc[j][v] = 0.f; }
        }
    }
}

template <int C, bool EXACT = false>
__global__ void __launch_bounds__(256, 4)
composite_bwd(int W, int H, int bg_len, const uint32_t *__restrict__ ranges, const uint32_t *__restrict__ point_list,
              const float *__restrict__ geom, const Feat colors, const float *__restrict__ bg,
              const float *__restrict__ final_T, const int32_t *__restrict__ n_contrib,
              const float *__restrict__ dL_dcolor, const float *__restrict__ dL_dallmap, float *__restrict__ grad_rec,
              const uint8_t *__restrict__ contrib_mask)
{
    constexpr int V = 15 + C;
    __shared__ TileLds<C, BWD_BATCH> lds;
    __shared__ float gacc[BWD_BATCH][V];
    __shared__ int s_max_last, s_dist;
    const int gx = (W + TILE - 1) / TILE, gy = (H + TILE - 1) / TILE;
    const int tile = xcd_tile(blockIdx.x, gx * gy);
    if (tile >= gx * gy) return;
    const int tx = tile % gx, ty = tile / gx;
    const int tid = threadIdx.x, wave = tid >> 6, lane = tid & 63;
    const int pxi = tx * TILE + (wave & 1) * 8 + (lane & 7);
    const int pyi = ty * TILE + (wave >> 1) * 8 + (lane >> 3);
    const bool inside = pxi < W && pyi < H;
    const size_t HW = (size_t)H * W, pid = (size_t)(inside ? pyi : 0) * W + (inside ? pxi : 0);
    const int32_t last = inside ? n_contrib[pid] : 0;
    const bool reg = inside && dL_dallmap && dL_dallmap[6 * HW + pid] != 0.0f;

    if (tid == 0) { s_max_last = 0; s_dist = 0; }
    for (int i = tid; i < BWD_BATCH * V; i += 256) (&gacc[0][0])[i] = 0.f;
    __syncthreads();
    {
        int m = last;
        m = max(m, __shfl_xor(m, 1)); m = max(m, __shfl_xor(m, 2)); m = max(m, __shfl_xor(m, 4));
        m = max(m, __shfl_xor(m, 8)); m = max(m, __shfl_xor(m, 16)); m = max(m, __shfl_xor(m, 32));
        if (lane == 0) atomicMax(&s_max_last, m);
        const bool any_reg = __builtin_amdgcn_ballot_w64(reg) != 0;
        if (lane == 0 && any_reg) s_dist = 1;
    }
    __syncthreads();
    const int max_last = s_max_last;
    const uint32_t r0 = ranges[2 * tile];
    if (s_dist)
        composite_bwd_tile<C, true, EXACT>(lds, gacc, W, H, bg_len, point_list, geom, colors, bg, final_T, n_contrib, dL_dcolor, dL_dallmap, grad_rec, r0, tx, ty, max_last, contrib_mask);
    else
        composite_bwd_tile<C, false, EXACT>(lds, gacc, W, H, bg_len, point_list, geom, colors, bg, final_T, n_contrib, dL_dcolor, dL_dallmap, grad_rec, r0, tx, ty, max_last, contrib_mask);
}

template <int C>
static int run_fwd(const envgs_raster_cfg *cfg, const uint32_t *ranges, const uint32_t *point_list, const float *geom,
                   const float *colors, const float *bg, float *out_color, float *allmap, float *final_T,
                   int32_t *n_contrib, float *weight, uint8_t *audit_contrib, int audit_lmax, hipStream_t stream, int colors_f16, uint8_t *contrib_mask,
                   const uint8_t *audit_skip)
{
    const int gx = (cfg->width + TILE - 1) / TILE, gy = (cfg->height + TILE - 1) / TILE;
    ProfScope prof_(K_COMPOSITE_FWD, stream);
    const dim3 grid(8 * ((gx * gy + 7) / 8)), block(256);
    const Feat colors_{colors, colors_f16 != 0};
#ifdef ENVGS_DIAG
    if (debug_switch(ENVGS_DBG_RASTER_EXACT)) {
        if (audit_contrib)
            hipLaunchKernelGGL((composite_fwd<C, true, true>), grid, block, 0, stream, cfg->width, cfg->height, cfg->bg_len, ranges,
                               point_list, geom, colors_, bg, out_color, allmap, final_T, n_contrib, weight, audit_contrib, audit_lmax, contrib_mask, audit_skip);
        else
            hipLaunchKernelGGL((composite_fwd<C, false, true>), grid, block, 0, stream, cfg->width, cfg->height, cfg->bg_len, ranges,
                               point_list, geom, colors_, bg, out_color, allmap, final_T, n_contrib, weight, (uint8_t *)nullptr, 0, contrib_mask, (const uint8_t *)nullptr);
        ENVGS_CHECK_LAUNCH(cfg, stream);
        return 0;
    }
#endif
    if (audit_contrib)
        hipLaunchKernelGGL((composite_fwd<C, true>), grid, block, 0, stream, cfg->width, cfg->height, cfg->bg_len, ranges,
                           point_list, geom, colors_, bg, out_color, allmap, final_T, n_contrib, weight, audit_contrib, audit_lmax, contrib_mask, audit_skip);
    else
        hipLaunchKernelGGL((composite_fwd<C, false>), grid, block, 0, stream, cfg->width, cfg->height, cfg->bg_len, ranges,
                           point_list, geom, colors_, bg, out_color, allmap, final_T, n_contrib, weight, (uint8_t *)nullptr, 0, contrib_mask, (const uint8_t *)nullptr);
    ENVGS_CHECK_LAUNCH(cfg, stream);
    return 0;
}

int launch_render_fwd(const envgs_raster_cfg *cfg, const uint32_t *ranges, const uint32_t *point_list, const float *geom,
                      const float *colors, const float *bg, float *out_color, float *allmap, float *final_T,
                      int32_t *n_contrib, float *weight, hipStream_t stream, uint8_t *audit_contrib, int audit_lmax, int colors_f16, uint8_t *contrib_mask,
                      const uint8_t *audit_skip)
{
    if (cfg->P > 0) {
        hipError_t e = hipMemsetAsync(weight, 0, sizeof(float) * (size_t)cfg->P, stream);
        if (e != hipSuccess) return (int)e;
    }
    switch (cfg->channels) {
    case 3: return run_fwd<3>(cfg, ranges, point_list, geom, colors, bg, out_color, allmap, final_T, n_contrib, weight, audit_contrib, audit_lmax, stream, colors_f16, contrib_mask, audit_skip);
    case 5: return run_fwd<5>(cfg, ranges, point_list, geom, colors, bg, out_color, allmap, final_T, n_contrib, weight, audit_contrib, audit_lmax, stream, colors_f16, contrib_mask, audit_skip);
    case 7: return run_fwd<7>(cfg, ranges, point_list, geom, colors, bg, out_color, allmap, final_T, n_contrib, weight, audit_contrib, audit_lmax, stream, colors_f16, contrib_mask, audit_skip);
    default: return ENVGS_ERR_BAD_ARG;
    }
}

template <int C>
static int run_bwd(const envgs_raster_cfg *cfg, const uint32_t *ranges, const uint32_t *point_list, const float *geom,
                   const float *colors, const float *bg, const float *final_T, const int32_t *n_contrib,
                   const float *dL_dcolor, const float *dL_dallmap, float *grad_rec, hipStream_t stream, int colors_f16, const uint8_t *contrib_mask)
{
    const int gx = (cfg->width + TILE - 1) / TILE, gy = (cfg->height + TILE - 1) / TILE;
    ProfScope prof_(K_COMPOSITE_BWD, stream);
#ifdef ENVGS_DIAG
    if (debug_switch(ENVGS_DBG_RASTER_EXACT)) {
        hipLaunchKernelGGL((composite_bwd<C, true>), dim3(8 * ((gx * gy + 7) / 8)), dim3(256), 0, stream, cfg->width, cfg->height, cfg->bg_len, ranges,
                           point_list, geom, Feat{colors, colors_f16 != 0}, bg, final_T, n_contrib, dL_dcolor, dL_dallmap, grad_rec, contrib_mask);
        ENVGS_CHECK_LAUNCH(cfg, stream);
        return 0;
    }
#endif
    hipLaunchKernelGGL((composite_bwd<C, false>), dim3(8 * ((gx * gy + 7) / 8)), dim3(256), 0, stream, cfg->width, cfg->height, cfg->bg_len, ranges,
                       point_list, geom, Feat{colors, colors_f16 != 0}, bg, final_T, n_contrib, dL_dcolor, dL_dallmap, grad_rec, contrib_mask);
    ENVGS_CHECK_LAUNCH(cfg, stream);
    return 0;
}

int launch_render_bwd(const envgs_raster_cfg *cfg, const uint32_t *ranges, const uint32_t *point_list, const float *geom,
                      const float *colors, const float *bg, const float *final_T, const int32_t *n_contrib,
                      const float *dL_dcolor, const float *dL_dallmap, float *grad_rec, hipStream_t stream, int colors_f16, const uint8_t *contrib_mask)
{
    if (cfg->P <= 0) return 0;
    hipError_t e = hipMemsetAsync(grad_rec, 0, sizeof(float) * GREC * (size_t)cfg->P, stream);
    if (e != hipSuccess) return (int)e;
    switch (cfg->channels) {
    case 3: return run_bwd<3>(cfg, ranges, point_list, geom, colors, bg, final_T, n_contrib, dL_dcolor, dL_dallmap, grad_rec, stream, colors_f16, contrib_mask);
    case 5: return run_bwd<5>(cfg, ranges, point_list, geom, colors, bg, final_T, n_contrib, dL_dcolor, dL_dallmap, grad_rec, stream, colors_f16, contrib_mask);
    case 7: return run_bwd<7>(cfg, ranges, point_list, geom, colors, bg, final_T, n_contrib, dL_dcolor, dL_dallmap, grad_rec, stream, colors_f16, contrib_mask);
    default: return ENVGS_ERR_BAD_ARG;
    }
}

}
```

envgs_amd/raster.py:

```python
from typing import NamedTuple

import torch
from torch import nn

from . import _lib


LAST_STATS = {}


class GaussianRasterizationSettings(NamedTuple):
    image_height: int
    image_width: int
    tanfovx: float
    tanfovy: float
    bg: torch.Tensor
    scale_modifier: float
    viewmatrix: torch.Tensor
    projmatrix: torch.Tensor
    sh_degree: int
    campos: torch.Tensor
    prefiltered: bool
    debug: bool


def _f32c(t):
    if t is None:
        return None
    if t.dtype != torch.float32:
        t = t.float()
    return t.contiguous()


def _featc(t):
    if t is None:
        return None
    if t.dtype != torch.float16:
        return _f32c(t)
    return t.contiguous()


def _stream(dev):
    return _lib.c_void_p(torch.cuda.current_stream(dev).cuda_stream)


import weakref

_DEG_CACHE = {}


def sh_degree_of(deg):
    if not torch.is_tensor(deg):
        return int(deg)
    key = id(deg)
    hit = _DEG_CACHE.get(key)
    if hit is not None and hit[0]() is deg and hit[1] == deg._version:
        return hit[2]
    v = int(deg.reshape(-1)[0].item())
    if len(_DEG_CACHE) > 64:
        for k in [k for k, h in _DEG_CACHE.items() if h[0]() is None]:
            del _DEG_CACHE[k]
    _DEG_CACHE[key] = (weakref.ref(deg), deg._version, v)
    return v


SPECULATIVE_N = {"on": True}
_N_GUESS = {}
_N_MIRROR = {}


def _n_mirror(dev):
    m = _N_MIRROR.get(dev.index)
    if m is None:
        m = _N_MIRROR[dev.index] = dict(host=torch.empty(1, dtype=torch.int32).pin_memory(), event=torch.cuda.Event())
    return m


FEATURE_STORAGE = {"f16": False}


def _store(t):
    if t is not None and FEATURE_STORAGE["f16"] and t.dtype == torch.float32 and t.numel() > 0:
        return t.detach().half()
    return t


CONTRIB_MASK = {"on": True}


def _cfg(settings, P, C, sh_coeffs, bg_len, f16=False):
    deg = sh_degree_of(settings.sh_degree)
    return _lib.RasterCfg(P, deg, sh_coeffs, C, int(settings.image_width), int(settings.image_height), bg_len,
                          1 if settings.debug else 0, float(settings.scale_modifier), float(settings.tanfovx),
                          float(settings.tanfovy), 1 if f16 else 0)


def rasterize_forward(C, means3D, shs, colors_precomp, opacities, scales, rotations, cov3D_precomp, settings,
                      keep_binning=False):
    lib = _lib.load()
    dev = means3D.device
    if dev.type != "cuda":
        raise RuntimeError("envgs_amd rasterizer needs tensors on the GPU (got %s); there is no CPU path" % dev)
    P = means3D.shape[0]
    H, W = int(settings.image_height), int(settings.image_width)
    means3D = _f32c(means3D); opacities = _f32c(opacities)
    shs = _featc(shs); colors_precomp = _featc(colors_precomp)
    f16 = any(t is not None and t.dtype == torch.float16 for t in (shs, colors_precomp))
    scales = _f32c(scales); rotations = _f32c(rotations); cov3D_precomp = _f32c(cov3D_precomp)
    if shs is not None and C != 3:
        raise RuntimeError("in-kernel SH evaluation produces 3 channels; the %d-channel rasterizer needs colors_precomp" % C)
    if colors_precomp is not None and colors_precomp.shape[-1] != C:
        raise RuntimeError("colors_precomp has %d channels, this rasterizer composites %d" % (colors_precomp.shape[-1], C))
    bg = _f32c(settings.bg).reshape(-1).to(dev)
    view = _f32c(settings.viewmatrix).to(dev); proj = _f32c(settings.projmatrix).to(dev)
    campos = _f32c(settings.campos).reshape(-1).to(dev)
    sh_coeffs = 0 if shs is None else int(shs.shape[1])
    cfg = _cfg(settings, P, C, sh_coeffs, min(int(bg.numel()), C), f16)
    stream = _stream(dev)
    f32 = dict(dtype=torch.float32, device=dev)
    i32 = dict(dtype=torch.int32, device=dev)

    geom = torch.empty(P, 16, **f32)
    radii = torch.empty(P, **i32)
    tiles = torch.empty(P, **i32)
    offsets = torch.empty(P, **i32)
    rgb = torch.empty(P, 3, **f32) if shs is not None else None
    clamped = torch.empty(P, 3, dtype=torch.uint8, device=dev) if shs is not None else None
    scan_bytes = lib.envgs_raster_scan_temp_bytes(P)
    scan_temp = torch.empty(max(scan_bytes, 1), dtype=torch.uint8, device=dev)
    p = _lib.ptr
    tiles_n = ((W + 15) // 16) * ((H + 15) // 16)
    colors = rgb if shs is not None else colors_precomp
    out_color = torch.empty(C, H, W, **f32)
    allmap = torch.empty(7, H, W, **f32)
    final_T = torch.empty(3, H, W, **f32)
    n_contrib = torch.empty(2, H, W, **i32)
    weight = torch.empty(P, 1, **f32)
    ranges = torch.empty(tiles_n, 2, **i32)

    def bin_and_render(cap):
        pairs = torch.empty(max(cap, 1), dtype=torch.int64, device=dev)
        keys_s = torch.empty(max(cap, 1), dtype=torch.int64, device=dev) if keep_binning else None
        point_list = torch.empty(max(cap, 1), **i32)
        bin_bytes = lib.envgs_raster_sort_temp_bytes(max(cap, 1), W, H)
        bin_temp = torch.empty(max(bin_bytes, 1), dtype=torch.uint8, device=dev)
        cmask = torch.empty(max(cap, 1), dtype=torch.uint8, device=dev) if CONTRIB_MASK["on"] else None
        _lib.check(lib.envgs_raster_bin_and_render(cfg, cap, p(geom), p(radii), p(colors), p(bg), p(pairs), p(keys_s), p(point_list),
                                                   p(bin_temp), bin_bytes, p(ranges), p(out_color), p(allmap), p(final_T),
                                                   p(n_contrib), p(weight), p(cmask), stream),
                   "envgs_raster_bin_and_render")
        return pairs, keys_s, point_list, cmask

    key = (dev.index, P, H, W)
    guess = _N_GUESS.get(key) if SPECULATIVE_N["on"] else None
    mirror = _n_mirror(dev)
    if guess is None or P == 0:
        n_host = _lib.c_uint32(0)
        _lib.check(lib.envgs_raster_project(cfg, p(means3D), p(scales), p(rotations), p(opacities), p(shs), p(cov3D_precomp),
                                            p(view), p(proj), p(campos), p(geom), p(rgb), p(clamped), p(radii), p(tiles),
                                            p(offsets), p(scan_temp), scan_bytes, n_host, stream), "envgs_raster_project")
        N = int(n_host.value)
        bufs = bin_and_render(N)
    else:
        _lib.check(lib.envgs_raster_project(cfg, p(means3D), p(scales), p(rotations), p(opacities), p(shs), p(cov3D_precomp),
                                            p(view), p(proj), p(campos), p(geom), p(rgb), p(clamped), p(radii), p(tiles),
                                            p(offsets), p(scan_temp), scan_bytes, None, stream), "envgs_raster_project")
        mirror["host"].copy_(offsets[P - 1:P], non_blocking=True)
        mirror["event"].record(torch.cuda.current_stream(dev))
        cap = guess
        bufs = bin_and_render(cap)
        mirror["event"].synchronize()
        N = int(mirror["host"][0]) & 0xFFFFFFFF
        if N > cap:
            LAST_STATS["n_guess_misses"] = LAST_STATS.get("n_guess_misses", 0) + 1
            bufs = bin_and_render(N)
    pairs, keys_s, point_list, cmask = bufs
    _N_GUESS[key] = max(((max(int(N * 1.15), N + 4096) + 65535) // 65536) * 65536, int(0.97 * (guess or 0)))
    LAST_STATS.update(N=N, P=P, H=H, W=W, C=C)
    saved = dict(cfg=cfg, N=N, geom=geom, colors=colors, bg=bg, point_list=point_list, ranges=ranges, final_T=final_T,
                 n_contrib=n_contrib, contrib_mask=cmask, means3D=means3D, scales=scales, rotations=rotations, shs=shs, clamped=clamped,
                 cov3D_precomp=cov3D_precomp, radii=radii, view=view, proj=proj, campos=campos)
    if keep_binning:
        saved.update(tiles_touched=tiles, offsets=offsets, tile_pairs=pairs, keys_sorted=keys_s)
    return (out_color, radii, allmap, weight), saved


def render_audit(saved, lmax, skip_px=None, want_weight=False):
    lib = _lib.load()
    cfg = saved["cfg"]
    dev = saved["geom"].device
    H, W, C, P = cfg.height, cfg.width, cfg.channels, cfg.P
    f32 = dict(dtype=torch.float32, device=dev)
    out_color = torch.empty(C, H, W, **f32); allmap = torch.empty(7, H, W, **f32); final_T = torch.empty(3, H, W, **f32)
    n_contrib = torch.empty(2, H, W, dtype=torch.int32, device=dev); weight = torch.empty(max(P, 1), **f32)
    contrib = torch.empty(H * W, int(lmax), dtype=torch.uint8, device=dev)
    skip = None if skip_px is None else skip_px.to(device=dev, dtype=torch.uint8).reshape(-1).contiguous()
    if skip is not None and skip.numel() != H * W:
        raise RuntimeError("skip_px must have H*W elements")
    p = _lib.ptr
    _lib.check(lib.envgs_raster_render_audit(cfg, p(saved["geom"]), p(saved["colors"]), p(saved["bg"]), p(saved["point_list"]),
                                             p(saved["ranges"]), p(out_color), p(allmap), p(final_T), p(n_contrib), p(weight),
                                             p(contrib), int(lmax), p(skip), _stream(dev)), "envgs_raster_render_audit")
    if want_weight:
        return contrib, n_contrib, out_color, weight[:P]
    return contrib, n_contrib, out_color


def rasterize_backward(saved, dL_dcolor, dL_dallmap):
    lib = _lib.load()
    cfg = saved["cfg"]
    P, C = cfg.P, cfg.channels
    dev = saved["geom"].device
    f32 = dict(dtype=torch.float32, device=dev)
    dL_dcolor = _f32c(dL_dcolor); dL_dallmap = _f32c(dL_dallmap)
    shs, cov = saved["shs"], saved["cov3D_precomp"]
    grad_rec = torch.empty(P, 32, **f32)
    dmeans3D = torch.empty(P, 3, **f32)
    dmeans2D = torch.empty(P, 3, **f32)
    dopac = torch.empty(P, 1, **f32)
    dscales = torch.empty(P, 2, **f32) if cov is None else None
    drots = torch.empty(P, 4, **f32) if cov is None else None
    dcov = torch.empty(P, 9, **f32) if cov is not None else None
    dshs = torch.empty(shs.shape, **f32) if shs is not None else None
    dcolors = torch.empty(P, C, **f32) if shs is None else None
    p = _lib.ptr
    _lib.check(lib.envgs_raster_backward(cfg, saved["N"], p(saved["geom"]), p(saved["colors"]), p(saved["bg"]),
                                         p(saved["point_list"]), p(saved["ranges"]), p(saved["final_T"]), p(saved["n_contrib"]),
                                         p(saved.get("contrib_mask")), p(dL_dcolor), p(dL_dallmap), p(saved["means3D"]), p(saved["scales"]), p(saved["rotations"]),
                                         p(shs), p(saved["clamped"]), p(cov), p(saved["radii"]), p(saved["view"]), p(saved["proj"]),
                                         p(saved["campos"]), p(grad_rec), p(dmeans3D), p(dmeans2D), p(dscales), p(drots), p(dshs),
                                         p(dcolors), p(dopac), p(dcov), _stream(dev)), "envgs_raster_backward")
    return dict(means3D=dmeans3D, means2D=dmeans2D, shs=dshs, colors_precomp=dcolors, opacities=dopac, scales=dscales,
                rotations=drots, cov3D_precomp=dcov, grad_rec=grad_rec)


def make_package(C):

    class _RasterizeGaussians(torch.autograd.Function):
        @staticmethod
        def forward(ctx, means3D, means2D, sh, colors_precomp, opacities, scales, rotations, cov3Ds_precomp, raster_settings):
            ctx.set_materialize_grads(False)
            none = lambda t: None if (t is None or t.numel() == 0) else t
            outs, saved = rasterize_forward(C, means3D, _store(none(sh)), _store(none(colors_precomp)), opacities, none(scales),
                                            none(rotations), none(cov3Ds_precomp), raster_settings)
            ctx.saved = saved
            ctx.in_dtypes = tuple(None if t is None else t.dtype for t in (means3D, means2D, sh, colors_precomp, opacities, scales, rotations, cov3Ds_precomp))
            color, radii, allmap, weight = outs
            ctx.mark_non_differentiable(radii, weight)
            return color, radii, allmap, weight

        @staticmethod
        def backward(ctx, grad_color, grad_radii, grad_allmap, grad_weight):
            saved = ctx.saved
            cfg = saved["cfg"]
            dev = saved["geom"].device
            g = rasterize_backward(saved, grad_color, grad_allmap)
            outs = (g["means3D"] if saved["cov3D_precomp"] is None or saved["shs"] is not None else None, g["means2D"],
                    g["shs"], g["colors_precomp"], g["opacities"], g["scales"], g["rotations"], g["cov3D_precomp"])
            outs = tuple(None if (o is None or dt is None) else o.to(dt) for o, dt in zip(outs, ctx.in_dtypes))
            return outs + (None,)

    class GaussianRasterizer(nn.Module):
        def __init__(self, raster_settings):
            super().__init__()
            self.raster_settings = raster_settings

        def markVisible(self, positions):
            with torch.no_grad():
                V = self.raster_settings.viewmatrix.to(positions.device).float()
                z = positions.float() @ V[:3, 2] + V[3, 2]
                return z > 0.2

        def forward(self, means3D, means2D, opacities, shs=None, colors_precomp=None, scales=None, rotations=None,
                    cov3D_precomp=None):
            rs = self.raster_settings
            if (shs is None and colors_precomp is None) or (shs is not None and colors_precomp is not None):
                raise Exception('Please provide excatly one of either SHs or precomputed colors!')
            if ((scales is None or rotations is None) and cov3D_precomp is None) or \
               ((scales is not None or rotations is not None) and cov3D_precomp is not None):
                raise Exception('Please provide exactly one of either scale/rotation pair or precomputed 3D covariance!')
            e = torch.Tensor([])
            return _RasterizeGaussians.apply(means3D, means2D, e if shs is None else shs,
                                             e if colors_precomp is None else colors_precomp, opacities,
                                             e if scales is None else scales, e if rotations is None else rotations,
                                             e if cov3D_precomp is None else cov3D_precomp, rs)

    GaussianRasterizer.channels = C
    GaussianRasterizer._function = _RasterizeGaussians
    return GaussianRasterizationSettings, GaussianRasterizer
```

include/envgs_raster.h:

```cpp
#ifndef ENVGS_RASTER_H
#define ENVGS_RASTER_H

#include <stddef.h>
#include <stdint.h>

#ifdef __cplusplus
extern "C" {
#endif

#if defined(__GNUC__)
#define ENVGS_API __attribute__((visibility("default")))
#else
#define ENVGS_API
#endif

#define ENVGS_TILE 16
#define ENVGS_GEOM_STRIDE 16
#define ENVGS_GRAD_STRIDE 32

typedef enum envgs_status {
    ENVGS_OK = 0,
    ENVGS_ERR_BAD_ARG = -1,
    ENVGS_ERR_TEMP_TOO_SMALL = -2
} envgs_status;

typedef struct envgs_raster_cfg {
    int32_t P;
    int32_t sh_degree;
    int32_t sh_coeffs;
    int32_t channels;
    int32_t width, height;
    int32_t bg_len;
    int32_t debug;
    float scale_modifier;
    float tanfovx, tanfovy;
    int32_t feature_f16;
} envgs_raster_cfg;

ENVGS_API size_t envgs_raster_scan_temp_bytes(int32_t P);
ENVGS_API size_t envgs_raster_sort_temp_bytes(uint32_t N, int32_t width, int32_t height);

ENVGS_API int envgs_raster_project(const envgs_raster_cfg *cfg,
                         const float *means3D, const float *scales, const float *rotations,
                         const float *opacities, const float *shs, const float *transmat_precomp,
                         const float *viewmatrix, const float *projmatrix, const float *campos,
                         float *geom, float *rgb, uint8_t *clamped, int32_t *radii,
                         uint32_t *tiles_touched, uint32_t *offsets,
                         void *scan_temp, size_t scan_temp_bytes,
                         uint32_t *num_rendered_host, void *stream);

ENVGS_API int envgs_raster_bin_and_render(const envgs_raster_cfg *cfg, uint32_t N,
                                const float *geom, const int32_t *radii,
                                const float *colors, const float *bg,
                                uint64_t *tile_pairs, uint64_t *keys_sorted , uint32_t *point_list,
                                void *bin_temp, size_t bin_temp_bytes, uint32_t *ranges,
                                float *out_color, float *allmap, float *final_T, int32_t *n_contrib,
                                float *weight, uint8_t *contrib_mask, void *stream);

ENVGS_API int envgs_raster_render_audit(const envgs_raster_cfg *cfg, const float *geom, const float *colors, const float *bg,
                              const uint32_t *point_list, const uint32_t *ranges,
                              float *out_color, float *allmap, float *final_T, int32_t *n_contrib, float *weight,
                              uint8_t *contrib, int32_t lmax, const uint8_t *skip_px, void *stream);

ENVGS_API int envgs_raster_backward(const envgs_raster_cfg *cfg, uint32_t N,
                          const float *geom, const float *colors, const float *bg,
                          const uint32_t *point_list, const uint32_t *ranges,
                          const float *final_T, const int32_t *n_contrib, const uint8_t *contrib_mask ,
                          const float *dL_dcolor, const float *dL_dallmap,
                          const float *means3D, const float *scales, const float *rotations,
                          const float *shs, const uint8_t *clamped, const float *transmat_precomp,
                          const int32_t *radii,
                          const float *viewmatrix, const float *projmatrix, const float *campos,
                          float *grad_rec,
                          float *dmeans3D, float *dmeans2D, float *dscales, float *drots,
                          float *dshs, float *dcolors, float *dopacities, float *dtransmat_precomp,
                          void *stream);

ENVGS_API void envgs_prof_enable(int on);
ENVGS_API void envgs_prof_select(uint64_t kernel_mask);
ENVGS_API int envgs_prof_read(int kernel_id, double *total_ms, int *launches);
ENVGS_API const char *envgs_prof_kernel_name(int kernel_id);

#define ENVGS_DBG_TRACE 0
#define ENVGS_DBG_SEGMENTS 1
#define ENVGS_DBG_COLLECT_WGS 2
#define ENVGS_DBG_RASTER_EXACT 3
#define ENVGS_DBG_RAYKEY 4
#define ENVGS_DBG_SPARSE 5
#define ENVGS_DBG_BALANCE 6
#define ENVGS_DBG_COUNT 7
ENVGS_API void envgs_debug_set(int32_t which, int32_t value);
ENVGS_API int32_t envgs_debug_get(int32_t which);

#ifdef __cplusplus
}
#endif
#endif
```

profiles/sched_model.py:

```python
import argparse
import heapq
import os
import sys

if __name__ == "__main__":
    sys.path[:] = [p for p in sys.path if os.path.abspath(p or ".") != os.path.dirname(os.path.abspath(__file__))]

import numpy as np


def makespan(workgroup_costs, slots=2048, xcds=8):
    per = max(1, slots // xcds)
    end = 0.0
    for x in range(xcds):
        mine = workgroup_costs[x::xcds]
        free = [0.0] * per
        heapq.heapify(free)
        for c in mine:
            t = heapq.heappop(free) + float(c)
            heapq.heappush(free, t)
            end = max(end, t)
    return end


def ideal(costs, slots=2048):
    costs = np.asarray(costs, dtype=np.float64)
    return max(costs.sum() / slots, costs.max() if costs.size else 0.0)


def strided_workgroups(costs, grid=8192):
    costs = np.asarray(costs, dtype=np.float64)
    g = min(grid, len(costs))
    out = np.zeros(g)
    for s in range(0, len(costs), g):
        part = costs[s:s + g]
        out[:len(part)] += part
    return out


def class_order(counts, classes):
    counts = np.asarray(counts, dtype=np.int64)
    key = counts if classes <= 0 else (counts * classes) // (int(counts.max()) + 1)
    return np.argsort(-key, kind="stable")


def report(counts, slots=2048, fixed=0.0):
    counts = np.asarray(counts, dtype=np.int64)
    if counts.ndim == 2:
        counts = counts.sum(1)
    cost = counts.astype(np.float64) + fixed
    lo = ideal(cost, slots)
    rows = [("coherence order, 8192 workgroups (round 6)", makespan(strided_workgroups(cost), slots) / lo)]
    for k in (1, 8, 32, 0):
        rows.append(("one workgroup per batch, %s" % ("full sort" if k == 0 else "K = %d" % k), makespan(cost[class_order(counts, k)], slots) / lo))
    return dict(batches=int(counts.size), mean=float(counts.mean()), cv=float(counts.std() / max(counts.mean(), 1e-9)), max=int(counts.max()),
                min=int(counts.min()), rounds=float(counts.size / slots), rows=rows)


def format_report(r):
    s = "batches %d  entries per batch: mean %.1f  cv %.3f  min %d  max %d  (%.2f rounds of the resident slots)\n" % (
        r["batches"], r["mean"], r["cv"], r["min"], r["max"], r["rounds"])
    for name, v in r["rows"]:
        s += "    %-46s makespan / ideal %.3f\n" % (name, v)
    return s


if __name__ == "__main__":
    ap = argparse.ArgumentParser()
    ap.add_argument("counts")
    ap.add_argument("--slots", type=int, default=2048, help="resident workgroups: 256 CUs x 4 SIMDs x 2 wavefronts")
    ap.add_argument("--fixed", type=float, default=0.0, help="cost of a batch beyond its entries, in entries")
    a = ap.parse_args()
    print(format_report(report(np.load(a.counts), a.slots, a.fixed)), end="")
```

Before: 137.9.

## Schedule raster tiles by cost classes for forward and backward render

Adds a tile-order schedule for rasterization. The scatter pass builds a forward order from per-tile instance counts, grouped into cost classes. The forward render records per-tile cost, and the backward render uses that cost to build its own order instead of the fixed XCD band mapping. The aim is to cut load-imbalance tail time across XCDs, at the cost of an extra workgroup, a schedule buffer and an indirection per workgroup. The Python path passes a tile_sched buffer to the new entry points.

```diff
diff --git a/envgs_amd/_lib.py b/envgs_amd/_lib.py
--- a/envgs_amd/_lib.py
+++ b/envgs_amd/_lib.py
@@ -104,8 +104,10 @@
     "envgs_raster_sort_temp_bytes": (c_size_t, [c_uint32, ctypes.c_int32, ctypes.c_int32]),
     "envgs_raster_project": (c_int, [ctypes.POINTER(RasterCfg)] + [_P] * 15 + [_P, c_size_t, ctypes.POINTER(c_uint32), _P]),
     "envgs_raster_bin_and_render": (c_int, [ctypes.POINTER(RasterCfg), c_uint32] + [_P] * 7 + [_P, c_size_t] + [_P] * 7 + [_P]),
+    "envgs_raster_bin_and_render_sched": (c_int, [ctypes.POINTER(RasterCfg), c_uint32] + [_P] * 7 + [_P, c_size_t] + [_P] * 8 + [_P]),
     "envgs_raster_render_audit": (c_int, [ctypes.POINTER(RasterCfg)] + [_P] * 11 + [ctypes.c_int32, _P, _P]),
     "envgs_raster_backward": (c_int, [ctypes.POINTER(RasterCfg), c_uint32] + [_P] * 29 + [_P]),
+    "envgs_raster_backward_sched": (c_int, [ctypes.POINTER(RasterCfg), c_uint32] + [_P] * 30 + [_P]),
     "envgs_bvh_temp_bytes": (c_size_t, [ctypes.c_int32]),
     "envgs_bvh_node_floats": (c_size_t, [ctypes.c_int32]),
     "envgs_bvh_build": (c_int, [ctypes.c_int32, _P, _P, _P, _P, c_size_t, ctypes.c_int32, _P]),
diff --git a/envgs_amd/csrc/common.h b/envgs_amd/csrc/common.h
--- a/envgs_amd/csrc/common.h
+++ b/envgs_amd/csrc/common.h
@@ -139,7 +139,8 @@
 size_t scan_temp_bytes(int n);
 size_t sort_temp_bytes(uint32_t n, int width, int height);
 int launch_bin(const envgs_raster_cfg *cfg, uint32_t N, const float *geom, const int32_t *radii, uint64_t *tile_pairs,
-               uint64_t *keys_sorted, uint32_t *point_list, void *bin_temp, size_t bin_temp_bytes, uint32_t *ranges, hipStream_t stream);
+               uint64_t *keys_sorted, uint32_t *point_list, void *bin_temp, size_t bin_temp_bytes, uint32_t *ranges, hipStream_t stream,
+               uint32_t *order_fwd = nullptr);
 size_t key_sort_temp_bytes(int n);
 int launch_key_sort(int n, const uint64_t *keys_in, uint64_t *keys_out, int top_bit, void *temp, size_t temp_bytes, hipStream_t stream);
 size_t ray_sort_temp_bytes(int R);
@@ -148,11 +149,12 @@
 int launch_render_fwd(const envgs_raster_cfg *cfg, const uint32_t *ranges, const uint32_t *point_list, const float *geom,
                       const float *colors, const float *bg, float *out_color, float *allmap, float *final_T,
                       int32_t *n_contrib, float *weight, hipStream_t stream, uint8_t *audit_contrib = nullptr, int audit_lmax = 0, int colors_f16 = 0,
-                      uint8_t *contrib_mask = nullptr, const uint8_t *audit_skip = nullptr);
+                      uint8_t *contrib_mask = nullptr, const uint8_t *audit_skip = nullptr, const uint32_t *order_fwd = nullptr,
+                      uint32_t *tile_cost_bwd = nullptr);
 int launch_render_bwd(const envgs_raster_cfg *cfg, const uint32_t *ranges, const uint32_t *point_list, const float *geom,
                       const float *colors, const float *bg, const float *final_T, const int32_t *n_contrib,
                       const float *dL_dcolor, const float *dL_dallmap, float *grad_rec, hipStream_t stream, int colors_f16 = 0,
-                      const uint8_t *contrib_mask = nullptr);
+                      const uint8_t *contrib_mask = nullptr, const uint32_t *tile_cost_bwd = nullptr, uint32_t *order_bwd = nullptr);
 int launch_project_bwd(const envgs_raster_cfg *cfg, const float *geom, const float *means3D, const float *scales,
                        const float *rotations, const float *shs, const uint8_t *clamped, const float *transmat_precomp,
                        const int32_t *radii, const float *viewmatrix, const float *projmatrix, const float *campos,
diff --git a/envgs_amd/csrc/raster_api.hip b/envgs_amd/csrc/raster_api.hip
--- a/envgs_amd/csrc/raster_api.hip
+++ b/envgs_amd/csrc/raster_api.hip
@@ -47,10 +47,10 @@
     return (int)e;
 }
 
-int envgs_raster_bin_and_render(const envgs_raster_cfg *cfg, uint32_t N, const float *geom, const int32_t *radii,
-                                const float *colors, const float *bg, uint64_t *tile_pairs, uint64_t *keys_sorted, uint32_t *point_list,
-                                void *bin_temp, size_t bin_temp_bytes_, uint32_t *ranges, float *out_color, float *allmap,
-                                float *final_T, int32_t *n_contrib, float *weight, uint8_t *contrib_mask, void *stream_)
+int envgs_raster_bin_and_render_sched(const envgs_raster_cfg *cfg, uint32_t N, const float *geom, const int32_t *radii,
+                                      const float *colors, const float *bg, uint64_t *tile_pairs, uint64_t *keys_sorted, uint32_t *point_list,
+                                      void *bin_temp, size_t bin_temp_bytes_, uint32_t *ranges, float *out_color, float *allmap,
+                                      float *final_T, int32_t *n_contrib, float *weight, uint8_t *contrib_mask, uint32_t *tile_sched, void *stream_)
 {
     int rc = check_cfg(cfg);
     if (rc) return rc;
@@ -58,10 +58,21 @@
     if (cfg->P > 0 && (!geom || !radii || !colors || !weight)) return ENVGS_ERR_BAD_ARG;
     if (N > 0 && (!tile_pairs || !point_list || !bin_temp)) return ENVGS_ERR_BAD_ARG;
     hipStream_t stream = (hipStream_t)stream_;
-    rc = launch_bin(cfg, N, geom, radii, tile_pairs, keys_sorted, point_list, bin_temp, bin_temp_bytes_, ranges, stream);
+    const size_t ntiles = (size_t)((cfg->width + TILE - 1) / TILE) * ((cfg->height + TILE - 1) / TILE);
+    uint32_t *order_fwd = tile_sched, *cost_bwd = tile_sched ? tile_sched + ntiles : nullptr;
+    rc = launch_bin(cfg, N, geom, radii, tile_pairs, keys_sorted, point_list, bin_temp, bin_temp_bytes_, ranges, stream, order_fwd);
     if (rc) return rc;
     return launch_render_fwd(cfg, ranges, point_list, geom, colors, bg, out_color, allmap, final_T, n_contrib, weight, stream, nullptr, 0,
-                             (cfg->feature_f16 && cfg->sh_coeffs == 0) ? 1 : 0, contrib_mask);
+                             (cfg->feature_f16 && cfg->sh_coeffs == 0) ? 1 : 0, contrib_mask, nullptr, order_fwd, cost_bwd);
+}
+
+int envgs_raster_bin_and_render(const envgs_raster_cfg *cfg, uint32_t N, const float *geom, const int32_t *radii,
+                                const float *colors, const float *bg, uint64_t *tile_pairs, uint64_t *keys_sorted, uint32_t *point_list,
+                                void *bin_temp, size_t bin_temp_bytes_, uint32_t *ranges, float *out_color, float *allmap,
+                                float *final_T, int32_t *n_contrib, float *weight, uint8_t *contrib_mask, void *stream_)
+{
+    return envgs_raster_bin_and_render_sched(cfg, N, geom, radii, colors, bg, tile_pairs, keys_sorted, point_list, bin_temp, bin_temp_bytes_, ranges,
+                                             out_color, allmap, final_T, n_contrib, weight, contrib_mask, nullptr, stream_);
 }
 
 int envgs_raster_render_audit(const envgs_raster_cfg *cfg, const float *geom, const float *colors, const float *bg,
@@ -79,14 +90,14 @@
                              (cfg->feature_f16 && cfg->sh_coeffs == 0) ? 1 : 0, nullptr, skip_px);
 }
 
-int envgs_raster_backward(const envgs_raster_cfg *cfg, uint32_t N, const float *geom, const float *colors, const float *bg,
-                          const uint32_t *point_list, const uint32_t *ranges, const float *final_T,
-                          const int32_t *n_contrib, const uint8_t *contrib_mask, const float *dL_dcolor, const float *dL_dallmap, const float *means3D,
-                          const float *scales, const float *rotations, const float *shs, const uint8_t *clamped,
-                          const float *transmat_precomp, const int32_t *radii, const float *viewmatrix,
-                          const float *projmatrix, const float *campos, float *grad_rec, float *dmeans3D, float *dmeans2D,
-                          float *dscales, float *drots, float *dshs, float *dcolors, float *dopacities,
-                          float *dtransmat_precomp, void *stream_)
+int envgs_raster_backward_sched(const envgs_raster_cfg *cfg, uint32_t N, const float *geom, const float *colors, const float *bg,
+                                const uint32_t *point_list, const uint32_t *ranges, const float *final_T,
+                                const int32_t *n_contrib, const uint8_t *contrib_mask, uint32_t *tile_sched, const float *dL_dcolor, const float *dL_dallmap,
+                                const float *means3D, const float *scales, const float *rotations, const float *shs, const uint8_t *clamped,
+                                const float *transmat_precomp, const int32_t *radii, const float *viewmatrix,
+                                const float *projmatrix, const float *campos, float *grad_rec, float *dmeans3D, float *dmeans2D,
+                                float *dscales, float *drots, float *dshs, float *dcolors, float *dopacities,
+                                float *dtransmat_precomp, void *stream_)
 {
     int rc = check_cfg(cfg);
     if (rc) return rc;
@@ -98,12 +109,28 @@
     if (shs ? (!dshs || !clamped || !campos || !means3D) : !dcolors) return ENVGS_ERR_BAD_ARG;
     if (transmat_precomp ? !dtransmat_precomp : (!scales || !rotations || !means3D || !dmeans3D || !dscales || !drots)) return ENVGS_ERR_BAD_ARG;
     hipStream_t stream = (hipStream_t)stream_;
+    const size_t ntiles = (size_t)((cfg->width + TILE - 1) / TILE) * ((cfg->height + TILE - 1) / TILE);
     rc = launch_render_bwd(cfg, ranges, point_list, geom, colors, bg, final_T, n_contrib, dL_dcolor, dL_dallmap, grad_rec, stream,
-                           (cfg->feature_f16 && !shs) ? 1 : 0, contrib_mask);
+                           (cfg->feature_f16 && !shs) ? 1 : 0, contrib_mask, tile_sched ? tile_sched + ntiles : nullptr,
+                           tile_sched ? tile_sched + 2 * ntiles : nullptr);
     if (rc) return rc;
     return launch_project_bwd(cfg, geom, means3D, scales, rotations, shs, clamped, transmat_precomp, radii, viewmatrix,
                               projmatrix, campos, grad_rec, dmeans3D, dmeans2D, dscales, drots, dshs, dcolors, dopacities,
                               dtransmat_precomp, stream);
 }
 
+int envgs_raster_backward(const envgs_raster_cfg *cfg, uint32_t N, const float *geom, const float *colors, const float *bg,
+                          const uint32_t *point_list, const uint32_t *ranges, const float *final_T,
+                          const int32_t *n_contrib, const uint8_t *contrib_mask, const float *dL_dcolor, const float *dL_dallmap, const float *means3D,
+                          const float *scales, const float *rotations, const float *shs, const uint8_t *clamped,
+                          const float *transmat_precomp, const int32_t *radii, const float *viewmatrix,
+                          const float *projmatrix, const float *campos, float *grad_rec, float *dmeans3D, float *dmeans2D,
+                          float *dscales, float *drots, float *dshs, float *dcolors, float *dopacities,
+                          float *dtransmat_precomp, void *stream_)
+{
+    return envgs_raster_backward_sched(cfg, N, geom, colors, bg, point_list, ranges, final_T, n_contrib, contrib_mask, nullptr, dL_dcolor, dL_dallmap,
+                                       means3D, scales, rotations, shs, clamped, transmat_precomp, radii, viewmatrix, projmatrix, campos, grad_rec,
+                                       dmeans3D, dmeans2D, dscales, drots, dshs, dcolors, dopacities, dtransmat_precomp, stream_);
 }
+
+}
diff --git a/envgs_amd/csrc/raster_bin.hip b/envgs_amd/csrc/raster_bin.hip
--- a/envgs_amd/csrc/raster_bin.hip
+++ b/envgs_amd/csrc/raster_bin.hip
@@ -1,6 +1,7 @@
 #include "common.h"
 #include "ray_key.h"
 #include "tile_sort.h"
+#include "tile_order.h"
 
 namespace envgs {
 
@@ -131,12 +132,17 @@
 template <bool SCATTER>
 __global__ void __launch_bounds__(256)
 bin_pass(int P, int W, int H, int slice, int ntiles, const float *__restrict__ geom, const int32_t *__restrict__ radii,
-         uint32_t *hist, const uint32_t *__restrict__ tile_start, uint64_t *__restrict__ pairs, uint32_t cap)
+         uint32_t *hist, const uint32_t *__restrict__ tile_start, uint64_t *__restrict__ pairs, uint32_t cap, uint32_t *__restrict__ order_fwd)
 {
     extern __shared__ uint32_t s_bin[];
+    if (SCATTER && order_fwd && blockIdx.x == 0) {
+        build_tile_order([&](int t) { return tile_start[t + 1] - tile_start[t]; }, ntiles, order_fwd);
+        return;
+    }
+    const int slice_id = (int)blockIdx.x - ((SCATTER && order_fwd) ? 1 : 0);
     const int gx = (W + TILE - 1) / TILE;
-    const int g0 = blockIdx.x * slice, g1 = min(P, g0 + slice);
-    uint32_t *row = hist + (size_t)blockIdx.x * ntiles;
+    const int g0 = slice_id * slice, g1 = min(P, g0 + slice);
+    uint32_t *row = hist + (size_t)slice_id * ntiles;
     const int lane = lane_id();
     for (int band0 = 0; band0 < ntiles; band0 += BIN_BAND) {
         const int bn = min(BIN_BAND, ntiles - band0);
@@ -428,11 +434,22 @@
     return cached[dev];
 }
 
+__global__ void __launch_bounds__(256)
+tile_order_identity(int ntiles, uint32_t *__restrict__ order_fwd)
+{
+    const int t = blockIdx.x * 256 + threadIdx.x;
+    if (t < ntiles) order_fwd[t] = (uint32_t)t;
+}
+
 int launch_bin(const envgs_raster_cfg *cfg, uint32_t N, const float *geom, const int32_t *radii, uint64_t *tile_pairs,
-               uint64_t *keys_sorted, uint32_t *point_list, void *bin_temp, size_t bin_temp_bytes, uint32_t *ranges, hipStream_t stream)
+               uint64_t *keys_sorted, uint32_t *point_list, void *bin_temp, size_t bin_temp_bytes, uint32_t *ranges, hipStream_t stream,
+               uint32_t *order_fwd)
 {
     const BinPlan pl = bin_plan(cfg->P, cfg->width, cfg->height);
-    if (N == 0 || cfg->P <= 0) return (int)hipMemsetAsync(ranges, 0, sizeof(uint32_t) * 2 * (size_t)pl.ntiles, stream);
+    if (N == 0 || cfg->P <= 0) {
+        if (order_fwd) hipLaunchKernelGGL(tile_order_identity, dim3((pl.ntiles + 255) / 256), dim3(256), 0, stream, pl.ntiles, order_fwd);
+        return (int)hipMemsetAsync(ranges, 0, sizeof(uint32_t) * 2 * (size_t)pl.ntiles, stream);
+    }
     if (bin_temp_bytes < sort_temp_bytes(N, cfg->width, cfg->height)) return ENVGS_ERR_TEMP_TOO_SMALL;
     uint32_t *hist = (uint32_t *)bin_temp;
     uint32_t *tile_count = hist + (size_t)BIN_ROWS_MAX * pl.ntiles;
@@ -442,14 +459,14 @@
     const size_t lds = sizeof(uint32_t) * (size_t)(pl.ntiles < BIN_BAND ? pl.ntiles : BIN_BAND);
     prof_begin(K_EMIT_KEYS, stream);
     hipLaunchKernelGGL(bin_pass<false>, dim3(pl.rows), dim3(256), lds, stream, cfg->P, cfg->width, cfg->height, pl.slice, pl.ntiles,
-                       geom, radii, hist, (const uint32_t *)nullptr, (uint64_t *)nullptr, 0u);
+                       geom, radii, hist, (const uint32_t *)nullptr, (uint64_t *)nullptr, 0u, (uint32_t *)nullptr);
     ENVGS_CHECK_LAUNCH(cfg, stream);
     hipLaunchKernelGGL(bin_column_scan, dim3((pl.ntiles + 15) / 16), dim3(256), 0, stream, pl.rows, pl.ntiles, hist, tile_count);
     ENVGS_CHECK_LAUNCH(cfg, stream);
     hipLaunchKernelGGL(bin_tile_scan, dim3(1), dim3(1024), 0, stream, pl.ntiles, tile_count, tile_start, ranges, N, hdr);
     ENVGS_CHECK_LAUNCH(cfg, stream);
-    hipLaunchKernelGGL(bin_pass<true>, dim3(pl.rows), dim3(256), lds, stream, cfg->P, cfg->width, cfg->height, pl.slice, pl.ntiles,
-                       geom, radii, hist, tile_start, tile_pairs, N);
+    hipLaunchKernelGGL(bin_pass<true>, dim3(pl.rows + (order_fwd ? 1 : 0)), dim3(256), lds, stream, cfg->P, cfg->width, cfg->height, pl.slice, pl.ntiles,
+                       geom, radii, hist, tile_start, tile_pairs, N, order_fwd);
     ENVGS_CHECK_LAUNCH(cfg, stream);
     prof_end(K_EMIT_KEYS, stream);
     ProfScope prof_(K_SORT, stream);
diff --git a/envgs_amd/csrc/raster_render.hip b/envgs_amd/csrc/raster_render.hip
--- a/envgs_amd/csrc/raster_render.hip
+++ b/envgs_amd/csrc/raster_render.hip
@@ -1,4 +1,5 @@
 #include "common.h"
+#include "tile_order.h"
 
 namespace envgs {
 
@@ -60,6 +61,14 @@
 {
     const int per = (ntiles + 7) >> 3;
     return (b & 7) * per + (b >> 3);
+}
+
+__device__ __forceinline__ int tile_of_workgroup(const uint32_t *__restrict__ order, int b, int ntiles)
+{
+    if (!order) { const int t = xcd_tile(b, ntiles); return t < ntiles ? t : -1; }
+    if (b >= ntiles) return -1;
+    const uint32_t t = order[b];
+    return t < (uint32_t)ntiles ? (int)t : -1;
 }
 
 __device__ __forceinline__ uint32_t quadrant_mask(const float4 r0, const float4 r1, const float4 r2, const float4 r3, int tile_px, int tile_py)
@@ -128,14 +137,16 @@
               const float *__restrict__ geom, const Feat colors, const float *__restrict__ bg,
               float *__restrict__ out_color, float *__restrict__ allmap, float *__restrict__ final_T,
               int32_t *__restrict__ n_contrib, float *__restrict__ weight, uint8_t *__restrict__ audit_contrib, int audit_lmax,
-              uint8_t *__restrict__ contrib_mask, const uint8_t *__restrict__ audit_skip)
+              uint8_t *__restrict__ contrib_mask, const uint8_t *__restrict__ audit_skip, const uint32_t *__restrict__ order,
+              uint32_t *__restrict__ tile_cost_bwd)
 {
     __shared__ TileLds<C> lds;
+    __shared__ unsigned s_cost[4];
     __shared__ float wacc[256];
     __shared__ unsigned char cmk[256][4];
     const int gx = (W + TILE - 1) / TILE, gy = (H + TILE - 1) / TILE;
-    const int tile = xcd_tile(blockIdx.x, gx * gy);
-    if (tile >= gx * gy) return;
+    const int tile = tile_of_workgroup(order, blockIdx.x, gx * gy);
+    if (tile < 0) return;
     const int tx = tile % gx, ty = tile / gx;
     const int tid = threadIdx.x, wave = tid >> 6, lane = tid & 63;
     const int pxi = tx * TILE + (wave & 1) * 8 + (lane & 7);
@@ -143,6 +154,7 @@
     const bool inside = pxi < W && pyi < H;
     const float px = (float)pxi, py = (float)pyi;
     const uint32_t r0 = ranges[2 * tile], r1 = ranges[2 * tile + 1];
+    unsigned wcost = 0u;
 
     const bool wskip = AUDIT && audit_skip && inside && audit_skip[(size_t)pyi * W + pxi] != 0;
     bool done = !inside;
@@ -211,16 +223,22 @@
           }
         }
         __syncthreads();
+        unsigned v = 0u;
         if (tid < count) {
             const float ws = wacc[tid];
             if (ws != 0.0f) { atomic_add_f32(weight + lds.id[tid], ws); wacc[tid] = 0.f; }
-            if (contrib_mask) {
-                unsigned *cw = reinterpret_cast<unsigned *>(&cmk[0][0]) + tid;
-                const unsigned v = *cw;
-                contrib_mask[base + tid] = (uint8_t)((v & 1u) | ((v >> 7) & 2u) | ((v >> 14) & 4u) | ((v >> 21) & 8u));
-                if (v) *cw = 0u;
-            }
-        }
+            unsigned *cw = reinterpret_cast<unsigned *>(&cmk[0][0]) + tid;
+            v = *cw;
+            if (contrib_mask) contrib_mask[base + tid] = (uint8_t)((v & 1u) | ((v >> 7) & 2u) | ((v >> 14) & 4u) | ((v >> 21) & 8u));
+            if (v) *cw = 0u;
+        }
+#pragma unroll
+        for (int q = 0; q < 4; q++) wcost += (unsigned)__popcll(__builtin_amdgcn_ballot_w64((v >> (8 * q)) & 1u));
+    }
+    if (tile_cost_bwd) {
+        if (lane == 0) s_cost[wave] = wcost;
+        __syncthreads();
+        if (tid == 0) tile_cost_bwd[tile] = s_cost[0] + s_cost[1] + s_cost[2] + s_cost[3];
     }
 
     if (inside) {
@@ -392,15 +410,15 @@
               const float *__restrict__ geom, const Feat colors, const float *__restrict__ bg,
               const float *__restrict__ final_T, const int32_t *__restrict__ n_contrib,
               const float *__restrict__ dL_dcolor, const float *__restrict__ dL_dallmap, float *__restrict__ grad_rec,
-              const uint8_t *__restrict__ contrib_mask)
+              const uint8_t *__restrict__ contrib_mask, const uint32_t *__restrict__ order)
 {
     constexpr int V = 15 + C;
     __shared__ TileLds<C, BWD_BATCH> lds;
     __shared__ float gacc[BWD_BATCH][V];
     __shared__ int s_max_last, s_dist;
     const int gx = (W + TILE - 1) / TILE, gy = (H + TILE - 1) / TILE;
-    const int tile = xcd_tile(blockIdx.x, gx * gy);
-    if (tile >= gx * gy) return;
+    const int tile = tile_of_workgroup(order, blockIdx.x, gx * gy);
+    if (tile < 0) return;
     const int tx = tile % gx, ty = tile / gx;
     const int tid = threadIdx.x, wave = tid >> 6, lane = tid & 63;
     const int pxi = tx * TILE + (wave & 1) * 8 + (lane & 7);
@@ -430,11 +448,27 @@
         composite_bwd_tile<C, false, EXACT>(lds, gacc, W, H, bg_len, point_list, geom, colors, bg, final_T, n_contrib, dL_dcolor, dL_dallmap, grad_rec, r0, tx, ty, max_last, contrib_mask);
 }
 
+static bool fixed_tile_bands() { return (debug_switch(ENVGS_DBG_BALANCE) & 2) != 0; }
+
+constexpr int CLEAR_ITEMS = 1024;
+__global__ void __launch_bounds__(256)
+clear_grad_build_order(float4 *__restrict__ grad, size_t n4, const uint32_t *__restrict__ tile_cost, int ntiles, uint32_t *__restrict__ order)
+{
+    if (order && blockIdx.x == 0) {
+        build_tile_order([&](int t) { return tile_cost[t]; }, ntiles, order);
+        return;
+    }
+    const size_t base = (size_t)(blockIdx.x - (order ? 1u : 0u)) * CLEAR_ITEMS + threadIdx.x;
+#pragma unroll
+    for (int k = 0; k < CLEAR_ITEMS / 256; k++)
+        if (base + (size_t)k * 256 < n4) grad[base + (size_t)k * 256] = make_float4(0.f, 0.f, 0.f, 0.f);
+}
+
 template <int C>
 static int run_fwd(const envgs_raster_cfg *cfg, const uint32_t *ranges, const uint32_t *point_list, const float *geom,
                    const float *colors, const float *bg, float *out_color, float *allmap, float *final_T,
                    int32_t *n_contrib, float *weight, uint8_t *audit_contrib, int audit_lmax, hipStream_t stream, int colors_f16, uint8_t *contrib_mask,
-                   const uint8_t *audit_skip)
+                   const uint8_t *audit_skip, const uint32_t *order, uint32_t *tile_cost_bwd)
 {
     const int gx = (cfg->width + TILE - 1) / TILE, gy = (cfg->height + TILE - 1) / TILE;
     ProfScope prof_(K_COMPOSITE_FWD, stream);
@@ -444,20 +478,20 @@
     if (debug_switch(ENVGS_DBG_RASTER_EXACT)) {
         if (audit_contrib)
             hipLaunchKernelGGL((composite_fwd<C, true, true>), grid, block, 0, stream, cfg->width, cfg->height, cfg->bg_len, ranges,
-                               point_list, geom, colors_, bg, out_color, allmap, final_T, n_contrib, weight, audit_contrib, audit_lmax, contrib_mask, audit_skip);
+                               point_list, geom, colors_, bg, out_color, allmap, final_T, n_contrib, weight, audit_contrib, audit_lmax, contrib_mask, audit_skip, order, tile_cost_bwd);
         else
             hipLaunchKernelGGL((composite_fwd<C, false, true>), grid, block, 0, stream, cfg->width, cfg->height, cfg->bg_len, ranges,
-                               point_list, geom, colors_, bg, out_color, allmap, final_T, n_contrib, weight, (uint8_t *)nullptr, 0, contrib_mask, (const uint8_t *)nullptr);
+                               point_list, geom, colors_, bg, out_color, allmap, final_T, n_contrib, weight, (uint8_t *)nullptr, 0, contrib_mask, (const uint8_t *)nullptr, order, tile_cost_bwd);
         ENVGS_CHECK_LAUNCH(cfg, stream);
         return 0;
     }
 #endif
     if (audit_contrib)
         hipLaunchKernelGGL((composite_fwd<C, true>), grid, block, 0, stream, cfg->width, cfg->height, cfg->bg_len, ranges,
-                           point_list, geom, colors_, bg, out_color, allmap, final_T, n_contrib, weight, audit_contrib, audit_lmax, contrib_mask, audit_skip);
+                           point_list, geom, colors_, bg, out_color, allmap, final_T, n_contrib, weight, audit_contrib, audit_lmax, contrib_mask, audit_skip, order, tile_cost_bwd);
     else
         hipLaunchKernelGGL((composite_fwd<C, false>), grid, block, 0, stream, cfg->width, cfg->height, cfg->bg_len, ranges,
-                           point_list, geom, colors_, bg, out_color, allmap, final_T, n_contrib, weight, (uint8_t *)nullptr, 0, contrib_mask, (const uint8_t *)nullptr);
+                           point_list, geom, colors_, bg, out_color, allmap, final_T, n_contrib, weight, (uint8_t *)nullptr, 0, contrib_mask, (const uint8_t *)nullptr, order, tile_cost_bwd);
     ENVGS_CHECK_LAUNCH(cfg, stream);
     return 0;
 }
@@ -465,16 +499,17 @@
 int launch_render_fwd(const envgs_raster_cfg *cfg, const uint32_t *ranges, const uint32_t *point_list, const float *geom,
                       const float *colors, const float *bg, float *out_color, float *allmap, float *final_T,
                       int32_t *n_contrib, float *weight, hipStream_t stream, uint8_t *audit_contrib, int audit_lmax, int colors_f16, uint8_t *contrib_mask,
-                      const uint8_t *audit_skip)
-{
+                      const uint8_t *audit_skip, const uint32_t *order_fwd, uint32_t *tile_cost_bwd)
+{
+    const uint32_t *order = fixed_tile_bands() ? nullptr : order_fwd;
     if (cfg->P > 0) {
         hipError_t e = hipMemsetAsync(weight, 0, sizeof(float) * (size_t)cfg->P, stream);
         if (e != hipSuccess) return (int)e;
     }
     switch (cfg->channels) {
-    case 3: return run_fwd<3>(cfg, ranges, point_list, geom, colors, bg, out_color, allmap, final_T, n_contrib, weight, audit_contrib, audit_lmax, stream, colors_f16, contrib_mask, audit_skip);
-    case 5: return run_fwd<5>(cfg, ranges, point_list, geom, colors, bg, out_color, allmap, final_T, n_contrib, weight, audit_contrib, audit_lmax, stream, colors_f16, contrib_mask, audit_skip);
-    case 7: return run_fwd<7>(cfg, ranges, point_list, geom, colors, bg, out_color, allmap, final_T, n_contrib, weight, audit_contrib, audit_lmax, stream, colors_f16, contrib_mask, audit_skip);
+    case 3: return run_fwd<3>(cfg, ranges, point_list, geom, colors, bg, out_color, allmap, final_T, n_contrib, weight, audit_contrib, audit_lmax, stream, colors_f16, contrib_mask, audit_skip, order, tile_cost_bwd);
+    case 5: return run_fwd<5>(cfg, ranges, point_list, geom, colors, bg, out_color, allmap, final_T, n_contrib, weight, audit_contrib, audit_lmax, stream, colors_f16, contrib_mask, audit_skip, order, tile_cost_bwd);
+    case 7: return run_fwd<7>(cfg, ranges, point_list, geom, colors, bg, out_color, allmap, final_T, n_contrib, weight, audit_contrib, audit_lmax, stream, colors_f16, contrib_mask, audit_skip, order, tile_cost_bwd);
     default: return ENVGS_ERR_BAD_ARG;
     }
 }
@@ -482,35 +517,43 @@
 template <int C>
 static int run_bwd(const envgs_raster_cfg *cfg, const uint32_t *ranges, const uint32_t *point_list, const float *geom,
                    const float *colors, const float *bg, const float *final_T, const int32_t *n_contrib,
-                   const float *dL_dcolor, const float *dL_dallmap, float *grad_rec, hipStream_t stream, int colors_f16, const uint8_t *contrib_mask)
+                   const float *dL_dcolor, const float *dL_dallmap, float *grad_rec, hipStream_t stream, int colors_f16, const uint8_t *contrib_mask,
+                   const uint32_t *order)
 {
     const int gx = (cfg->width + TILE - 1) / TILE, gy = (cfg->height + TILE - 1) / TILE;
+    const dim3 grid(8 * ((gx * gy + 7) / 8));
     ProfScope prof_(K_COMPOSITE_BWD, stream);
 #ifdef ENVGS_DIAG
     if (debug_switch(ENVGS_DBG_RASTER_EXACT)) {
-        hipLaunchKernelGGL((composite_bwd<C, true>), dim3(8 * ((gx * gy + 7) / 8)), dim3(256), 0, stream, cfg->width, cfg->height, cfg->bg_len, ranges,
-                           point_list, geom, Feat{colors, colors_f16 != 0}, bg, final_T, n_contrib, dL_dcolor, dL_dallmap, grad_rec, contrib_mask);
+        hipLaunchKernelGGL((composite_bwd<C, true>), grid, dim3(256), 0, stream, cfg->width, cfg->height, cfg->bg_len, ranges,
+                           point_list, geom, Feat{colors, colors_f16 != 0}, bg, final_T, n_contrib, dL_dcolor, dL_dallmap, grad_rec, contrib_mask, order);
         ENVGS_CHECK_LAUNCH(cfg, stream);
         return 0;
     }
 #endif
-    hipLaunchKernelGGL((composite_bwd<C, false>), dim3(8 * ((gx * gy + 7) / 8)), dim3(256), 0, stream, cfg->width, cfg->height, cfg->bg_len, ranges,
-                       point_list, geom, Feat{colors, colors_f16 != 0}, bg, final_T, n_contrib, dL_dcolor, dL_dallmap, grad_rec, contrib_mask);
+    hipLaunchKernelGGL((composite_bwd<C, false>), grid, dim3(256), 0, stream, cfg->width, cfg->height, cfg->bg_len, ranges,
+                       point_list, geom, Feat{colors, colors_f16 != 0}, bg, final_T, n_contrib, dL_dcolor, dL_dallmap, grad_rec, contrib_mask, order);
     ENVGS_CHECK_LAUNCH(cfg, stream);
     return 0;
 }
 
 int launch_render_bwd(const envgs_raster_cfg *cfg, const uint32_t *ranges, const uint32_t *point_list, const float *geom,
                       const float *colors, const float *bg, const float *final_T, const int32_t *n_contrib,
-                      const float *dL_dcolor, const float *dL_dallmap, float *grad_rec, hipStream_t stream, int colors_f16, const uint8_t *contrib_mask)
+                      const float *dL_dcolor, const float *dL_dallmap, float *grad_rec, hipStream_t stream, int colors_f16, const uint8_t *contrib_mask,
+                      const uint32_t *tile_cost_bwd, uint32_t *order_bwd)
 {
     if (cfg->P <= 0) return 0;
-    hipError_t e = hipMemsetAsync(grad_rec, 0, sizeof(float) * GREC * (size_t)cfg->P, stream);
-    if (e != hipSuccess) return (int)e;
+    if (!tile_cost_bwd) order_bwd = nullptr;
+    const int ntiles = ((cfg->width + TILE - 1) / TILE) * ((cfg->height + TILE - 1) / TILE);
+    const size_t n4 = (size_t)cfg->P * (GREC / 4);
+    hipLaunchKernelGGL(clear_grad_build_order, dim3((unsigned)((n4 + CLEAR_ITEMS - 1) / CLEAR_ITEMS) + (order_bwd ? 1u : 0u)), dim3(256), 0, stream,
+                       reinterpret_cast<float4 *>(grad_rec), n4, tile_cost_bwd, ntiles, order_bwd);
+    ENVGS_CHECK_LAUNCH(cfg, stream);
+    const uint32_t *order = fixed_tile_bands() ? nullptr : order_bwd;
     switch (cfg->channels) {
-    case 3: return run_bwd<3>(cfg, ranges, point_list, geom, colors, bg, final_T, n_contrib, dL_dcolor, dL_dallmap, grad_rec, stream, colors_f16, contrib_mask);
-    case 5: return run_bwd<5>(cfg, ranges, point_list, geom, colors, bg, final_T, n_contrib, dL_dcolor, dL_dallmap, grad_rec, stream, colors_f16, contrib_mask);
-    case 7: return run_bwd<7>(cfg, ranges, point_list, geom, colors, bg, final_T, n_contrib, dL_dcolor, dL_dallmap, grad_rec, stream, colors_f16, contrib_mask);
+    case 3: return run_bwd<3>(cfg, ranges, point_list, geom, colors, bg, final_T, n_contrib, dL_dcolor, dL_dallmap, grad_rec, stream, colors_f16, contrib_mask, order);
+    case 5: return run_bwd<5>(cfg, ranges, point_list, geom, colors, bg, final_T, n_contrib, dL_dcolor, dL_dallmap, grad_rec, stream, colors_f16, contrib_mask, order);
+    case 7: return run_bwd<7>(cfg, ranges, point_list, geom, colors, bg, final_T, n_contrib, dL_dcolor, dL_dallmap, grad_rec, stream, colors_f16, contrib_mask, order);
     default: return ENVGS_ERR_BAD_ARG;
     }
 }
diff --git a/envgs_amd/csrc/tile_order.h b/envgs_amd/csrc/tile_order.h
--- /dev/null
+++ b/envgs_amd/csrc/tile_order.h
@@ -0,0 +1,74 @@
+#pragma once
+#include "common.h"
+
+namespace envgs {
+
+constexpr int TILE_ORDER_CLASSES = ENVGS_TILE_ORDER_CLASSES;
+constexpr int TILE_ORDER_SEGS = 4;
+constexpr unsigned TILE_COST_MAX = 1u << 26;
+
+__device__ __forceinline__ int tile_order_class(unsigned cost, unsigned maxc)
+{
+    cost = cost > maxc ? maxc : cost;
+    return TILE_ORDER_CLASSES - 1 - (int)((cost * (unsigned)TILE_ORDER_CLASSES) / (maxc + 1u));
+}
+
+template <class Cost>
+__device__ __forceinline__ void build_tile_order(const Cost cost_of, const int n, uint32_t *__restrict__ order)
+{
+    constexpr int K = TILE_ORDER_CLASSES, NB = 5;
+    static_assert((1 << NB) == K && (K * TILE_ORDER_SEGS) % 64 == 0, "class bits");
+    __shared__ unsigned s_off[K * TILE_ORDER_SEGS];
+    __shared__ unsigned s_max;
+    const int tid = threadIdx.x, lane = tid & 63, wave = tid >> 6;
+    const int seglen = (((n + TILE_ORDER_SEGS - 1) / TILE_ORDER_SEGS) + 63) & ~63;
+    auto cost = [&](int t) { const unsigned c = cost_of(t); return c > TILE_COST_MAX ? TILE_COST_MAX : c; };
+    if (tid == 0) s_max = 0u;
+    for (int i = tid; i < K * TILE_ORDER_SEGS; i += 256) s_off[i] = 0u;
+    __syncthreads();
+    unsigned m = 0u;
+#pragma unroll 4
+    for (int t = tid; t < n; t += 256) m = max(m, cost(t));
+    if (m > 0u) atomicMax(&s_max, m);
+    __syncthreads();
+    const unsigned maxc = s_max;
+#pragma unroll 4
+    for (int t = tid; t < n; t += 256) atomicAdd(&s_off[tile_order_class(cost(t), maxc) * TILE_ORDER_SEGS + t / seglen], 1u);
+    __syncthreads();
+    if (wave == 0) {
+        unsigned carry = 0u;
+        for (int k0 = 0; k0 < K * TILE_ORDER_SEGS; k0 += 64) {
+            const unsigned v = s_off[k0 + lane];
+            unsigned incl = v;
+#pragma unroll
+            for (int d = 1; d < 64; d <<= 1) { const unsigned o = __shfl_up(incl, d); if (lane >= d) incl += o; }
+            s_off[k0 + lane] = carry + incl - v;
+            carry += __shfl(incl, 63);
+        }
+    }
+    __syncthreads();
+    const int seg0 = wave * seglen, seg1 = min(seg0 + seglen, n);
+    unsigned next = seg0 + lane < seg1 ? cost(seg0 + lane) : 0u;
+    for (int t0 = seg0; t0 < seg1; t0 += 64) {
+        const int t = t0 + lane;
+        const bool act = t < seg1;
+        const unsigned c = next;
+        next = t + 64 < seg1 ? cost(t + 64) : 0u;
+        const int bin = act ? tile_order_class(c, maxc) : 0;
+        unsigned long long mask = __ballot(act);
+#pragma unroll
+        for (int bit = 0; bit < NB; bit++) {
+            const bool one = (bin >> bit) & 1;
+            const unsigned long long bb = __ballot(act && one);
+            mask &= one ? bb : ~bb;
+        }
+        const int rank = __popcll(mask & ((1ull << lane) - 1ull));
+        unsigned first = 0u;
+        if (act && rank == 0) first = atomicAdd(&s_off[bin * TILE_ORDER_SEGS + wave], (unsigned)__popcll(mask));
+        first = __shfl(first, act ? __ffsll((long long)mask) - 1 : lane);
+        if (act && first + (unsigned)rank < (unsigned)n) order[first + (unsigned)rank] = (uint32_t)t;
+    }
+}
+
+
+}
diff --git a/envgs_amd/raster.py b/envgs_amd/raster.py
--- a/envgs_amd/raster.py
+++ b/envgs_amd/raster.py
@@ -83,6 +83,15 @@
     if t is not None and FEATURE_STORAGE["f16"] and t.dtype == torch.float32 and t.numel() > 0:
         return t.detach().half()
     return t
+
+
+TILE_ORDER_CLASSES = 32
+
+
+def tile_order_class(costs, classes=TILE_ORDER_CLASSES):
+    import numpy as np
+    c = np.minimum(np.asarray(costs, dtype=np.int64), 1 << 26)
+    return (c * classes) // (int(c.max()) + 1 if c.size else 1)
 
 
 CONTRIB_MASK = {"on": True}
@@ -137,6 +146,7 @@
     n_contrib = torch.empty(2, H, W, **i32)
     weight = torch.empty(P, 1, **f32)
     ranges = torch.empty(tiles_n, 2, **i32)
+    tile_sched = torch.empty(3, tiles_n, **i32)
 
     def bin_and_render(cap):
         pairs = torch.empty(max(cap, 1), dtype=torch.int64, device=dev)
@@ -145,10 +155,10 @@
         bin_bytes = lib.envgs_raster_sort_temp_bytes(max(cap, 1), W, H)
         bin_temp = torch.empty(max(bin_bytes, 1), dtype=torch.uint8, device=dev)
         cmask = torch.empty(max(cap, 1), dtype=torch.uint8, device=dev) if CONTRIB_MASK["on"] else None
-        _lib.check(lib.envgs_raster_bin_and_render(cfg, cap, p(geom), p(radii), p(colors), p(bg), p(pairs), p(keys_s), p(point_list),
-                                                   p(bin_temp), bin_bytes, p(ranges), p(out_color), p(allmap), p(final_T),
-                                                   p(n_contrib), p(weight), p(cmask), stream),
-                   "envgs_raster_bin_and_render")
+        _lib.check(lib.envgs_raster_bin_and_render_sched(cfg, cap, p(geom), p(radii), p(colors), p(bg), p(pairs), p(keys_s), p(point_list),
+                                                         p(bin_temp), bin_bytes, p(ranges), p(out_color), p(allmap), p(final_T),
+                                                         p(n_contrib), p(weight), p(cmask), p(tile_sched), stream),
+                   "envgs_raster_bin_and_render_sched")
         return pairs, keys_s, point_list, cmask
 
     key = (dev.index, P, H, W)
@@ -178,7 +188,7 @@
     _N_GUESS[key] = max(((max(int(N * 1.15), N + 4096) + 65535) // 65536) * 65536, int(0.97 * (guess or 0)))
     LAST_STATS.update(N=N, P=P, H=H, W=W, C=C)
     saved = dict(cfg=cfg, N=N, geom=geom, colors=colors, bg=bg, point_list=point_list, ranges=ranges, final_T=final_T,
-                 n_contrib=n_contrib, contrib_mask=cmask, means3D=means3D, scales=scales, rotations=rotations, shs=shs, clamped=clamped,
+                 n_contrib=n_contrib, contrib_mask=cmask, tile_sched=tile_sched, means3D=means3D, scales=scales, rotations=rotations, shs=shs, clamped=clamped,
                  cov3D_precomp=cov3D_precomp, radii=radii, view=view, proj=proj, campos=campos)
     if keep_binning:
         saved.update(tiles_touched=tiles, offsets=offsets, tile_pairs=pairs, keys_sorted=keys_s)
@@ -224,12 +234,13 @@
     dshs = torch.empty(shs.shape, **f32) if shs is not None else None
     dcolors = torch.empty(P, C, **f32) if shs is None else None
     p = _lib.ptr
-    _lib.check(lib.envgs_raster_backward(cfg, saved["N"], p(saved["geom"]), p(saved["colors"]), p(saved["bg"]),
-                                         p(saved["point_list"]), p(saved["ranges"]), p(saved["final_T"]), p(saved["n_contrib"]),
-                                         p(saved.get("contrib_mask")), p(dL_dcolor), p(dL_dallmap), p(saved["means3D"]), p(saved["scales"]), p(saved["rotations"]),
-                                         p(shs), p(saved["clamped"]), p(cov), p(saved["radii"]), p(saved["view"]), p(saved["proj"]),
-                                         p(saved["campos"]), p(grad_rec), p(dmeans3D), p(dmeans2D), p(dscales), p(drots), p(dshs),
-                                         p(dcolors), p(dopac), p(dcov), _stream(dev)), "envgs_raster_backward")
+    _lib.check(lib.envgs_raster_backward_sched(cfg, saved["N"], p(saved["geom"]), p(saved["colors"]), p(saved["bg"]),
+                                               p(saved["point_list"]), p(saved["ranges"]), p(saved["final_T"]), p(saved["n_contrib"]),
+                                               p(saved.get("contrib_mask")), p(saved.get("tile_sched")), p(dL_dcolor), p(dL_dallmap), p(saved["means3D"]),
+                                               p(saved["scales"]), p(saved["rotations"]),
+                                               p(shs), p(saved["clamped"]), p(cov), p(saved["radii"]), p(saved["view"]), p(saved["proj"]),
+                                               p(saved["campos"]), p(grad_rec), p(dmeans3D), p(dmeans2D), p(dscales), p(drots), p(dshs),
+                                               p(dcolors), p(dopac), p(dcov), _stream(dev)), "envgs_raster_backward_sched")
     return dict(means3D=dmeans3D, means2D=dmeans2D, shs=dshs, colors_precomp=dcolors, opacities=dopac, scales=dscales,
                 rotations=drots, cov3D_precomp=dcov, grad_rec=grad_rec)
 
diff --git a/include/envgs_raster.h b/include/envgs_raster.h
--- a/include/envgs_raster.h
+++ b/include/envgs_raster.h
@@ -57,6 +57,15 @@
                                 float *out_color, float *allmap, float *final_T, int32_t *n_contrib,
                                 float *weight, uint8_t *contrib_mask, void *stream);
 
+#define ENVGS_TILE_ORDER_CLASSES 32
+ENVGS_API int envgs_raster_bin_and_render_sched(const envgs_raster_cfg *cfg, uint32_t N,
+                                const float *geom, const int32_t *radii,
+                                const float *colors, const float *bg,
+                                uint64_t *tile_pairs, uint64_t *keys_sorted , uint32_t *point_list,
+                                void *bin_temp, size_t bin_temp_bytes, uint32_t *ranges,
+                                float *out_color, float *allmap, float *final_T, int32_t *n_contrib,
+                                float *weight, uint8_t *contrib_mask, uint32_t *tile_sched, void *stream);
+
 ENVGS_API int envgs_raster_render_audit(const envgs_raster_cfg *cfg, const float *geom, const float *colors, const float *bg,
                               const uint32_t *point_list, const uint32_t *ranges,
                               float *out_color, float *allmap, float *final_T, int32_t *n_contrib, float *weight,
@@ -66,6 +75,21 @@
                           const float *geom, const float *colors, const float *bg,
                           const uint32_t *point_list, const uint32_t *ranges,
                           const float *final_T, const int32_t *n_contrib, const uint8_t *contrib_mask ,
+                          const float *dL_dcolor, const float *dL_dallmap,
+                          const float *means3D, const float *scales, const float *rotations,
+                          const float *shs, const uint8_t *clamped, const float *transmat_precomp,
+                          const int32_t *radii,
+                          const float *viewmatrix, const float *projmatrix, const float *campos,
+                          float *grad_rec,
+                          float *dmeans3D, float *dmeans2D, float *dscales, float *drots,
+                          float *dshs, float *dcolors, float *dopacities, float *dtransmat_precomp,
+                          void *stream);
+
+ENVGS_API int envgs_raster_backward_sched(const envgs_raster_cfg *cfg, uint32_t N,
+                          const float *geom, const float *colors, const float *bg,
+                          const uint32_t *point_list, const uint32_t *ranges,
+                          const float *final_T, const int32_t *n_contrib, const uint8_t *contrib_mask ,
+                          uint32_t *tile_sched,
                           const float *dL_dcolor, const float *dL_dallmap,
                           const float *means3D, const float *scales, const float *rotations,
                           const float *shs, const uint8_t *clamped, const float *transmat_precomp,
diff --git a/profiles/sched_model.py b/profiles/sched_model.py
--- a/profiles/sched_model.py
+++ b/profiles/sched_model.py
@@ -21,6 +21,67 @@
             heapq.heappush(free, t)
             end = max(end, t)
     return end
+
+
+def makespan_xcd(workgroup_costs, slots_per_xcd, rule="strict", xcds=8):
+    costs = [float(c) for c in workgroup_costs]
+    if rule == "strict":
+        return makespan(costs, slots_per_xcd * xcds, xcds)
+    if rule == "free":
+        return makespan(costs, slots_per_xcd * xcds, 1)
+    if rule != "blocking":
+        raise ValueError(rule)
+    free = [[0.0] * slots_per_xcd for _ in range(xcds)]
+    end = last_start = 0.0
+    for i, c in enumerate(costs):
+        q = free[i % xcds]
+        last_start = max(heapq.heappop(q), last_start)
+        heapq.heappush(q, last_start + c)
+        end = max(end, last_start + c)
+    return end
+
+
+def fixed_bands(costs, xcds=8):
+    costs = np.asarray(costs, dtype=np.float64)
+    per = (len(costs) + xcds - 1) // xcds
+    out = np.zeros(per * xcds)
+    for b in range(per * xcds):
+        t = (b % xcds) * per + b // xcds
+        if t < len(costs):
+            out[b] = costs[t]
+    return out
+
+
+def equal_cost_bands(counts, classes=32, xcds=8):
+    counts = np.asarray(counts, dtype=np.int64)
+    before = np.concatenate([[0], np.cumsum(counts)[:-1]])
+    total = max(int(counts.sum()), 1)
+    band = np.minimum((before * xcds) // total, xcds - 1) if counts.sum() > 0 else (np.arange(len(counts)) * xcds) // max(len(counts), 1)
+    members = [np.flatnonzero(band == x) for x in range(xcds)]
+    members = [m[class_order(counts[m], classes)] if m.size else m for m in members]
+    longest = max(m.size for m in members)
+    out = np.full(longest * xcds, -1, dtype=np.int64)
+    for x, m in enumerate(members):
+        out[x + xcds * np.arange(m.size)] = m
+    return out
+
+
+def report_tiles(counts, slots_per_xcd=128, fixed=0.0, classes=32):
+    counts = np.asarray(counts, dtype=np.int64)
+    cost = counts.astype(np.float64) + fixed
+    lo = ideal(cost, slots_per_xcd * 8)
+    eb = equal_cost_bands(counts, classes)
+    mappings = [("fixed bands (xcd_tile)", fixed_bands(cost)),
+                ("descending classes, K = %d" % classes, cost[class_order(counts, classes)]),
+                ("equal-cost bands, heaviest first (B)", np.where(eb >= 0, cost[np.maximum(eb, 0)], 0.0))]
+    return [(name, {rule: makespan_xcd(wg, slots_per_xcd, rule) / lo for rule in ("strict", "blocking", "free")}) for name, wg in mappings]
+
+
+def format_tiles(rows):
+    s = "    %-40s %8s %8s %8s\n" % ("makespan / ideal under rule:", "strict", "blocking", "free")
+    for name, r in rows:
+        s += "    %-40s %8.3f %8.3f %8.3f\n" % (name, r["strict"], r["blocking"], r["free"])
+    return s
 
 
 def ideal(costs, slots=2048):
@@ -67,8 +128,15 @@
 
 if __name__ == "__main__":
     ap = argparse.ArgumentParser()
-    ap.add_argument("counts")
+    ap.add_argument("counts", nargs="?")
+    ap.add_argument("--tiles", default=None, help="XCD mode: the (tiles, 3) per-tile array of balance_profile.py --save-counts")
+    ap.add_argument("--column", type=int, default=2, help="XCD mode: 0 instances (R6's cost), 1 contributing, 2 passes (R7's cost)")
+    ap.add_argument("--slots-per-xcd", type=int, default=128, help="XCD mode: resident workgroups per XCD (R7: 32 CUs x 4; R6: x 5 = 160)")
     ap.add_argument("--slots", type=int, default=2048, help="resident workgroups: 256 CUs x 4 SIMDs x 2 wavefronts")
     ap.add_argument("--fixed", type=float, default=0.0, help="cost of a batch beyond its entries, in entries")
     a = ap.parse_args()
+    if a.tiles:
+        t = np.load(a.tiles)
+        print(format_tiles(report_tiles(t[:, a.column] if t.ndim == 2 else t, a.slots_per_xcd, a.fixed)), end="")
+        sys.exit(0)
     print(format_report(report(np.load(a.counts), a.slots, a.fixed)), end="")
```

New measurement: 136.8. No clear change (-0.8%).
